# johnnyjana730/MVIN

Measured on AMD Instinct MI355X. Metric: (user,item) pairs scored/sec @ dim=64 hop=2 fan-out=32; % HBM roofline, higher is better.
Workload: dtype f32

## Files before the change

### mvin_amd/build.py

```python
import argparse
import hashlib
import os
import shutil
import subprocess
import sys

PKG_DIR = os.path.dirname(os.path.abspath(__file__))
CSRC = os.path.join(PKG_DIR, "csrc")
INCLUDE = os.path.join(os.path.dirname(PKG_DIR), "include")
LIB_PATH = os.path.join(PKG_DIR, "libmvin_hip.so")
STAMP_PATH = LIB_PATH + ".stamp"
OBJ_DIR = os.path.join(PKG_DIR, "_build")
SOURCES = ["mvin_kernels.hip", "mvin_fused.hip", "mvin_fused_split.hip", "mvin_fused_packed.hip", "mvin_fused_wpp.hip", "mvin_fused_agg.hip", "mvin_fused_agg32.hip", "mvin_fused_wpp_fold.hip", "mvin_fused_d16.hip", "mvin_fused_d32.hip", "mvin_tail.hip", "mvin_tail_flash.hip", "mvin_score_small.hip", "mvin_keyaddr.hip", "mvin_keyaddr_stream.hip", "mvin_keyaddr_grouped.hip", "mvin_keyaddr_dense.hip", "mvin_keyaddr_static.hip", "mvin_keyaddr_flash.hip", "mvin_keyaddr_wave.hip", "mvin_hoist.hip", "mvin_probe.hip", "mvin_group.hip", "mvin_order.hip", "mvin_topk.hip", "mvin_rank.hip", "mvin_segments.hip", "mvin_mmr.hip", "mvin_mips.hip", "mvin_resample.hip", "mvin_explore.hip", "mvin_ctr_metrics.hip", "mvin_ctr_delong.hip", "mvin_ctr_curve.hip", "mvin_ctr_rank_resample.hip","mvin_ctr_cluster.hip", "mvin_ctr_segments.hip", "mvin_ctr_calib.hip", "mvin_rank_head.hip", "mvin_mf.hip", "mvin_select_negatives.hip", "mvin_explain.hip", "mvin_explain_mem.hip", "mvin_prep.hip", "mvin_negatives.hip", "mvin_linear_mfma.hip", "mvin_entity_tables.hip", "mvin_bwd.hip", "mvin_grad_guard.hip",
           "mvin_abi_basic.hip", "mvin_abi_levels.hip", "mvin_abi_keyaddr.hip", "mvin_abi_score.hip", "mvin_abi_eval.hip", "mvin_abi_train.hip"]
HEADERS = ["mvin_common.h", "mvin_kernels.h", "mvin_launch.h", "mvin_fused_agg.h", "mvin_score_image.h", "mvin_ctr_bodies.h", "mvin_row_select.h", "mvin_rnd.h", "mvin_explain_mass.h", "mvin_rank_head_body.h",
           "mvin_workspaces.h", "mvin_score_plan.h", "mvin_abi_util.h", "mvin_entity_tables_plan.h", "mvin_l2_kernel_plan.h"]
VERSION_SCRIPT = os.path.join(CSRC, "libmvin_hip.map")
ARCH = "gfx950"
FLAGS = ["-O3", "-std=c++17", "-fPIC", "-fvisibility=hidden", "-shared", f"--offload-arch={ARCH}"]


def _hipcc():
    for cand in (os.environ.get("HIPCC"), shutil.which("hipcc"), "/opt/rocm/bin/hipcc"):
        if cand and os.path.exists(cand):
            return cand
    raise RuntimeError("hipcc not found (looked at $HIPCC, PATH, /opt/rocm/bin/hipcc)")


def _existing(names, base):
    return [os.path.join(base, n) for n in names if os.path.exists(os.path.join(base, n))]


def _digest():
    h = hashlib.sha256(" ".join(FLAGS).encode())
    for path in _existing(SOURCES + HEADERS, CSRC) + [os.path.join(INCLUDE, "mvin_hip.h"), VERSION_SCRIPT]:
        with open(path, "rb") as f:
            h.update(path.encode())
            h.update(f.read())
    return h.hexdigest()


def needs_build():
    if not os.path.exists(LIB_PATH) or not os.path.exists(STAMP_PATH):
        return True
    with open(STAMP_PATH) as f:
        return f.read().strip() != _digest()


def _obj_digest(src):
    h = hashlib.sha256(" ".join(FLAGS).encode())
    for path in [src] + _existing(HEADERS, CSRC) + [os.path.join(INCLUDE, "mvin_hip.h")]:
        with open(path, "rb") as f:
            h.update(f.read())
    return h.hexdigest()[:20]


def build(force=False, verbose=False, jobs=None):
    if not force and not needs_build():
        return LIB_PATH
    os.makedirs(OBJ_DIR, exist_ok=True)
    import fcntl
    with open(os.path.join(OBJ_DIR, ".lock"), "w") as lock:
        fcntl.flock(lock, fcntl.LOCK_EX)
        try:
            if not force and not needs_build():
                return LIB_PATH
            return _build_locked(force, verbose, jobs)
        finally:
            fcntl.flock(lock, fcntl.LOCK_UN)


def _build_locked(force, verbose, jobs):
    from concurrent.futures import ThreadPoolExecutor
    tmp_suffix = f".{os.getpid()}.tmp"
    hipcc = _hipcc()
    cflags = [f for f in FLAGS if f != "-shared"]
    todo, objs = [], []
    for src in _existing(SOURCES, CSRC):
        obj = os.path.join(OBJ_DIR, os.path.basename(src) + "." + _obj_digest(src) + ".o")
        objs.append(obj)
        if force or not os.path.exists(obj):
            todo.append((src, obj))

    def compile_one(job):
        src, obj = job
        cmd = [hipcc] + cflags + ["-c", f"-I{INCLUDE}", f"-I{CSRC}", src, "-o", obj + tmp_suffix]
        if verbose:
            print(" ".join(cmd), file=sys.stderr)
        res = subprocess.run(cmd, capture_output=True, text=True)
        if res.returncode != 0:
            raise RuntimeError(f"hipcc failed ({res.returncode}) on {src}:\n{res.stdout}\n{res.stderr}")
        if verbose and res.stderr:
            print(res.stderr, file=sys.stderr)
        os.replace(obj + tmp_suffix, obj)

    if todo:
        with ThreadPoolExecutor(max_workers=jobs or min(6, os.cpu_count() or 1)) as ex:
            list(ex.map(compile_one, todo))
    keep = set(objs)
    for f in os.listdir(OBJ_DIR):
        if os.path.join(OBJ_DIR, f) not in keep and not f.endswith(".tmp") and f != ".lock":
            os.remove(os.path.join(OBJ_DIR, f))
    cmd = [hipcc, "-shared", "-fPIC", f"--offload-arch={ARCH}", f"-Wl,--version-script={VERSION_SCRIPT}"] + objs + ["-o", LIB_PATH + tmp_suffix]
    res = subprocess.run(cmd, capture_output=True, text=True)
    if res.returncode != 0:
        raise RuntimeError(f"link failed ({res.returncode}):\n{res.stdout}\n{res.stderr}")
    os.replace(LIB_PATH + tmp_suffix, LIB_PATH)
    with open(STAMP_PATH, "w") as f:
        f.write(_digest())
    return LIB_PATH


if __name__ == "__main__":
    ap = argparse.ArgumentParser()
    ap.add_argument("--force", action="store_true")
    ap.add_argument("--verbose", action="store_true")
    a = ap.parse_args()
    print(build(force=a.force, verbose=a.verbose))
```

### mvin_amd/csrc/mvin_abi_keyaddr.hip

```cpp
#include "mvin_abi_util.h"

namespace mvin {
namespace abi {

int group_pairs_impl(const int64_t* users_i64, const int32_t* users_i32, int64_t B, int n_user, int32_t* workspace, int32_t* seg_user,
                     int32_t* seg_ptr, int32_t* nseg, int32_t* pair_index, void* stream, const int64_t* items64, unsigned max_id,
                     int32_t* item_rows) {
    const char* who = "mvin_group_pairs_by_user";
    if ((!users_i64 && !users_i32) || !workspace || !seg_user || !seg_ptr || !nseg || !pair_index)
        return fail(-1, "%s: null pointer", who);
    if (B <= 0 || B > 0x7fffffff || n_user <= 0) return fail(-2, "%s: bad sizes B=%lld n_user=%d", who, (long long)B, n_user);
    const GroupWs L(n_user, B);
    return hip_result(mvin::launch_group_pairs(users_i64, users_i32, B, n_user, workspace + L.counters(), workspace + L.offsets(),
                                               workspace + L.ranks(), seg_user, seg_ptr, nseg, pair_index, (hipStream_t)stream,
                                               reinterpret_cast<const int32_t*>(items64), 2, max_id, item_rows), who);
}

int flash_prepare_impl(const char* who, const float* entity_emb, const float* relation_kge, const float* w, const float* user_mlp_W, int n_entity,
                       int nR, int D, int P, float* ws, float* fold_ws, void* stream) {
    if (!entity_emb || !relation_kge || !user_mlp_W || !ws) return fail(-1, "%s: null pointer", who);
    if (n_entity <= 0 || nR <= 0 || D != 64 || P < 1 || P > 8) return fail(-2, "%s: n_entity=%d nR=%d D=%d P=%d", who, n_entity, nR, D, P);
    const RelWs L(n_entity, nR, D);
    if (int rc = build_entity_tables(who, entity_emb, n_entity, relation_kge, nR, ws + L.ER(), user_mlp_W, P + (w ? 1 : 0), ws + L.TW(),
                                     fold_ws ? fold_ws + FoldWs(n_entity, D).block() : nullptr, fold_ws, stream))
        return rc;
    if (w) return hip_result(mvin::launch_entity_dot(entity_emb, w, n_entity, D, ws + L.hs(), (hipStream_t)stream), who);
    return 0;
}

}
}

using namespace mvin::abi;

extern "C" {

int mvin_key_addressing_supported(int Nm, int D) {
    return (!bad_dim(D) && Nm > 0 && mvin::key_addr_nj(Nm, D) <= 16) ? 1 : 0;
}

static int key_addressing_impl(const char* who, const void* entity_emb, const float* V, const float* w,
                               const int32_t* const* mem_h, const int32_t* const* mem_r, const int32_t* const* mem_t,
                               const int32_t* uts, const int64_t* users64, const int32_t* users32, int P, int B, int Nm,
                               int D, int nR, int n_entity, int n_user, float* out, int64_t ldo, int table_bf16,
                               void* stream) {
    if (n_entity <= 0) return fail(-2, "%s: n_entity=%d", who, n_entity);
    if (uts && n_user <= 0) return fail(-2, "%s: n_user=%d", who, n_user);
    if (!entity_emb || !out || (!uts && !mem_h)) return fail(-1, "%s: null pointer", who);
    if (uts && !users64 && !users32) return fail(-1, "%s: user_triplet_set given without user ids", who);
    if (P < 0 || P > 8) return fail(-2, "%s: P=%d (0..8)", who, P);
    if (P == 0 && !w) return fail(-2, "%s: nothing to do (P == 0 and w == NULL)", who);
    if (P > 0 && (!V || nR <= 0 || (!uts && (!mem_r || !mem_t)))) return fail(-1, "%s: hops need V, mem_r, mem_t, nR", who);
    if (B <= 0 || Nm <= 0) return fail(-2, "%s: bad sizes B=%d Nm=%d", who, B, Nm);
    if (bad_dim(D)) return fail(-2, "%s: D=%d (need %%4==0, 4..%d)", who, D, MVIN_MAX_DIM);
    const int n_o = P + (w ? 1 : 0);
    if (ldo < (int64_t)n_o * D || (ldo & 3)) return fail(-2, "%s: ldo=%lld", who, (long long)ldo);
    mvin::KeyAddrArgs k{};
    k.E = entity_emb;
    k.V = V;
    k.w = w;
    k.uts = uts;
    k.users64 = users64;
    k.users32 = users32;
    k.n_user = n_user;
    k.n_entity = n_entity;
    const int nh = P > 0 ? P : 1;
    for (int i = 0; i < nh && !uts; ++i) {
        if (!mem_h[i]) return fail(-1, "%s: null mem_h[%d]", who, i);
        k.mem_h[i] = mem_h[i];
        if (i < P) {
            if (!mem_r[i] || !mem_t[i]) return fail(-1, "%s: null mem_r/mem_t[%d]", who, i);
            k.mem_r[i] = mem_r[i];
            k.mem_t[i] = mem_t[i];
        }
    }
    k.out = out;
    k.ldo = ldo;
    k.B = B;
    k.P = P;
    k.Nm = Nm;
    k.D = D;
    k.nR = nR;
    k.lpr_log2 = mvin::lpr_log2_for(D);
    k.table_bytes = (uint64_t)n_entity * D * (table_bf16 ? 2 : 4);
    if (!mvin::key_addr_stream_supported(k, table_bf16) && mvin::key_addr_nj(Nm, D) > 16)
        return fail(-3, "%s: unsupported shape Nm=%d D=%d (streaming kernel: Nm <= 64 and nR*D*4 <= 3072; "
                    "register-resident kernel: ceil(Nm / (64 / lanes per row)) <= 16)", who, Nm, D);
    return hip_result(mvin::launch_key_addr(k, table_bf16, (hipStream_t)stream), who);
}

int mvin_key_addressing_fwd(const void* entity_emb, const float* V, const float* w,
                            const int32_t* const* mem_h, const int32_t* const* mem_r,
                            const int32_t* const* mem_t, int P, int B, int Nm, int D, int nR, int n_entity,
                            float* out, int64_t ldo, int table_bf16, void* stream) {
    return key_addressing_impl("mvin_key_addressing_fwd", entity_emb, V, w, mem_h, mem_r, mem_t, nullptr, nullptr, nullptr, P,
                               B, Nm, D, nR, n_entity, 0, out, ldo, table_bf16, stream);
}

int mvin_key_addressing_users_fwd(const void* entity_emb, const float* V, const float* w, const int32_t* uts,
                                  const int64_t* users_i64, const int32_t* users_i32, int P, int B, int Nm, int D, int nR,
                                  int n_entity, int n_user, float* out, int64_t ldo, int table_bf16, void* stream) {
    return key_addressing_impl("mvin_key_addressing_users_fwd", entity_emb, V, w, nullptr, nullptr, nullptr, uts, users_i64,
                               users_i32, P, B, Nm, D, nR, n_entity, n_user, out, ldo, table_bf16, stream);
}

int mvin_group_pairs_by_user(const int64_t* users_i64, const int32_t* users_i32, int64_t B, int n_user, int32_t* workspace,
                             int32_t* seg_user, int32_t* seg_ptr, int32_t* nseg, int32_t* pair_index, void* stream) {
    return group_pairs_impl(users_i64, users_i32, B, n_user, workspace, seg_user, seg_ptr, nseg, pair_index, stream, nullptr, 0, nullptr);
}

int mvin_key_addressing_grouped_supported(int D, int P, int Nm, int nR) {
    return mvin::key_addr_grouped_supported(D, P, Nm, nR) ? 1 : 0;
}

int mvin_user_records_len(int P, int Nm, int nR) { return mvin::ka_rec_layout(P, Nm, nR).len; }

int mvin_user_records_supported(int D, int P, int Nm, int nR, int table_bf16) {
    return !table_bf16 && mvin::key_addr_static_supported(D, P, Nm, nR) ? 1 : 0;
}

int mvin_build_user_records(const int32_t* uts, int n_user, int P, int Nm, int nR, int n_entity, int32_t* records, void* stream) {
    const char* who = "mvin_build_user_records";
    if (!uts || !records) return fail(-1, "%s: null pointer", who);
    if (n_user <= 0 || n_entity <= 0) return fail(-2, "%s: bad sizes n_user=%d n_entity=%d", who, n_user, n_entity);
    if (mvin::ka_rec_layout(P, Nm, nR).len == 0) return fail(-3, "%s: no record form for P=%d Nm=%d nR=%d (P 1..8, Nm 1..256, nR 1..4096)", who, P, Nm, nR);
    return hip_result(mvin::launch_user_records(uts, n_user, P, Nm, nR, n_entity, records, (hipStream_t)stream), who);
}

int mvin_key_addressing_grouped_fwd(const void* entity_emb, const float* relation_kge, const float* w,
                                    const int32_t* uts, const int32_t* seg_user, const int32_t* seg_ptr,
                                    const int32_t* nseg_dev, const int32_t* pair_index, const int64_t* items_i64,
                                    const int32_t* items_i32, int nseg, int B, int P, int Nm, int D, int nR,
                                    int n_entity, int n_user, float* out, int64_t ldo, int table_bf16, void* stream) {
    return mvin_key_addressing_grouped_rec_fwd(entity_emb, relation_kge, w, uts, nullptr, seg_user, seg_ptr, nseg_dev, pair_index, items_i64,
                                               items_i32, nseg, B, P, Nm, D, nR, n_entity, n_user, out, ldo, table_bf16, stream);
}

size_t mvin_project_relations_elems(int n_entity, int nR, int D) {
    return n_entity > 0 && nR > 0 && D > 0 ? mvin::RelWs(n_entity, nR, D).elems() : 0;
}

int mvin_project_relations(const float* entity_emb, const float* relation_kge, const float* w, int n_entity, int nR, int D, float* ws,
                           void* stream) {
    const char* who = "mvin_project_relations";
    if (!entity_emb || !relation_kge || !ws) return fail(-1, "%s: null pointer", who);
    if (n_entity <= 0 || nR <= 0 || (D != 16 && D != 32 && D != 64 && D != 128)) return fail(-2, "%s: n_entity=%d nR=%d D=%d", who, n_entity, nR, D);
    const mvin::RelWs L(n_entity, nR, D);
    if (D == 64) {
        if (int rc = build_entity_tables(who, entity_emb, n_entity, relation_kge, nR, ws + L.ER(), nullptr, 0, nullptr, nullptr, nullptr, stream)) return rc;
    } else {
        float* RT = ws + L.RT();
        if (int rc = hip_result(mvin::launch_transpose_blocks(relation_kge, nR, D, RT, (hipStream_t)stream), who)) return rc;
        mvin_linear_args l{};
        l.src[0] = entity_emb;
        l.nsrc = 1;
        l.Dsrc = D;
        l.Dout = D;
        l.rows = n_entity;
        l.rows_per_group = 1;
        l.W = RT;
        l.w_zstride = (int64_t)L.DD;
        l.out = ws + L.ER();
        l.ldo = D;
        l.nz = nR;
        l.out_zstride = (int64_t)L.tab;
        if (int rc = mvin_linear_fwd(&l, stream)) return rc;
    }
    if (w) return hip_result(mvin::launch_entity_dot(entity_emb, w, n_entity, D, ws + L.hs(), (hipStream_t)stream), who);
    return 0;
}

int mvin_key_addressing_flash_supported(int D, int P, int Nm, int nR, int n_entity) {
    return mvin::key_addr_flash_supported(D, P, Nm, nR, n_entity) ? 1 : 0;
}

static int flash_nseg_bound(int64_t B, int n_user) { return (int)(B < (int64_t)n_user ? B : (int64_t)n_user); }

size_t mvin_key_addressing_flash_ws_elems(int64_t B, int n_user) {
    if (B <= 0 || n_user <= 0) return 0;
    return mvin::key_addr_flash_ws_elems(B, flash_nseg_bound(B, n_user));
}

size_t mvin_key_addressing_flash_tables_elems(int n_entity, int nR, int D, int P, int has_set) {
    if (n_entity <= 0 || nR <= 0 || D <= 0 || P < 0) return 0;
    return mvin::RelWs(n_entity, nR, D).flash_elems(P + (has_set ? 1 : 0));
}

int mvin_key_addressing_flash_prepare(const float* entity_emb, const float* relation_kge, const float* w, const float* user_mlp_W,
                                      int n_entity, int nR, int D, int P, float* ws, void* stream) {
    return flash_prepare_impl("mvin_key_addressing_flash_prepare", entity_emb, relation_kge, w, user_mlp_W, n_entity, nR, D, P, ws, nullptr,
                              stream);
}

int mvin_key_addressing_flash_fwd(const float* entity_emb, const float* ws, const int32_t* user_records, const int32_t* seg_user,
                                  const int32_t* seg_ptr, const int32_t* nseg_dev, const int32_t* pair_index, const int64_t* items_i64,
                                  const int32_t* items_i32, int64_t B, int P, int Nm, int D, int nR, int n_entity, int n_user, int has_set,
                                  const float* user_mlp_b, float* user_o, int32_t* sched_ws, void* stream) {
    const char* who = "mvin_key_addressing_flash_fwd";
    if (!entity_emb || !ws || !user_records || !seg_user || !seg_ptr || !pair_index || !user_o || !sched_ws)
        return fail(-1, "%s: null pointer", who);
    if ((items_i64 == nullptr) == (items_i32 == nullptr)) return fail(-1, "%s: exactly one of items_i64 / items_i32", who);
    if (B <= 0 || B >= (int64_t(1) << 31) || n_user <= 0 || n_entity <= 0 || nR <= 0)
        return fail(-2, "%s: bad sizes B=%lld n_user=%d n_entity=%d nR=%d", who, (long long)B, n_user, n_entity, nR);
    if (!mvin::key_addr_flash_supported(D, P, Nm, nR, n_entity))
        return fail(-3, "%s: unsupported shape D=%d P=%d Nm=%d nR=%d n_entity=%d (D = 64, 1 <= P <= 8, Nm <= 64, nR * n_entity < 2^31)", who,
                    D, P, Nm, nR, n_entity);
    mvin::KaFlashArgs k{};
    k.E = entity_emb;
    const mvin::RelWs L(n_entity, nR, D);
    k.ER = ws + L.ER();
    k.hs = has_set ? ws + L.hs() : nullptr;
    k.TW = ws + L.TW();
    k.records = user_records;
    k.seg_user = seg_user;
    k.seg_ptr = seg_ptr;
    k.nseg_dev = nseg_dev;
    k.pair_index = pair_index;
    k.items64 = items_i64;
    k.items32 = items_i32;
    k.bmlp = user_mlp_b;
    k.user_o = user_o;
    k.P = P;
    k.Nm = Nm;
    k.nR = nR;
    k.n_entity = n_entity;
    k.B = B;
    return hip_result(mvin::launch_key_addr_flash(k, flash_nseg_bound(B, n_user), has_set != 0, sched_ws, (hipStream_t)stream), who);
}

static int key_addressing_grouped_impl(const void* entity_emb, const float* relation_kge, const float* w,
                                        const int32_t* uts, const int32_t* user_records, const int32_t* seg_user,
                                        const int32_t* seg_ptr, const int32_t* nseg_dev, const int32_t* pair_index,
                                        const int64_t* items_i64, const int32_t* items_i32, int nseg, int B, int P, int Nm, int D,
                                        int nR, int n_entity, int n_user, float* out, int64_t ldo, int table_bf16, void* stream,
                                        const float* er_ws) {
    const char* who = "mvin_key_addressing_grouped_fwd";
    if (!entity_emb || !uts || !seg_user || !seg_ptr || !pair_index || !out) return fail(-1, "%s: null pointer", who);
    if ((items_i64 == nullptr) == (items_i32 == nullptr)) return fail(-1, "%s: exactly one of items_i64 / items_i32", who);
    if (P < 0 || P > 8) return fail(-2, "%s: P=%d (0..8)", who, P);
    if (P == 0 && !w) return fail(-2, "%s: nothing to do (P == 0 and w == NULL)", who);
    if (P > 0 && !relation_kge) return fail(-1, "%s: hops need relation_kge", who);
    if (nseg <= 0 || B <= 0 || Nm <= 0 || n_entity <= 0 || n_user <= 0 || nR <= 0)
        return fail(-2, "%s: bad sizes nseg=%d B=%d Nm=%d n_entity=%d n_user=%d nR=%d", who, nseg, B, Nm, n_entity, n_user, nR);
    const int n_o = P + (w ? 1 : 0);
    if (ldo < (int64_t)n_o * D || (ldo & 3)) return fail(-2, "%s: ldo=%lld", who, (long long)ldo);
    if (!mvin::key_addr_grouped_supported(D, P, Nm, nR))
        return fail(-3, "%s: unsupported shape D=%d P=%d Nm=%d nR=%d (D in {16,32,64,128}; rows + V tile must fit 160 KB "
                    "of LDS)", who, D, P, Nm, nR);
    mvin::KeyAddrGroupedArgs k{};
    k.E = entity_emb;
    k.R = relation_kge;
    k.w = w;
    k.uts = uts;
    k.seg_user = seg_user;
    k.seg_ptr = seg_ptr;
    k.nseg_dev = nseg_dev;
    k.pair_index = pair_index;
    k.items64 = items_i64;
    k.items32 = items_i32;
    k.out = out;
    k.ldo = ldo;
    k.nseg = nseg;
    k.P = P;
    k.Nm = Nm;
    k.D = D;
    k.nR = nR;
    k.n_entity = n_entity;
    k.records = user_records;
    if (er_ws) {
        const mvin::RelWs L(n_entity, nR, D);
        k.ER = er_ws + L.ER();
        k.hs = er_ws + L.hs();
    }
    return hip_result(mvin::launch_key_addr_grouped(k, table_bf16, (hipStream_t)stream), who);
}

int mvin_key_addressing_grouped_rec_fwd(const void* entity_emb, const float* relation_kge, const float* w,
                                        const int32_t* uts, const int32_t* user_records, const int32_t* seg_user,
                                        const int32_t* seg_ptr, const int32_t* nseg_dev, const int32_t* pair_index,
                                        const int64_t* items_i64, const int32_t* items_i32, int nseg, int B, int P, int Nm, int D,
                                        int nR, int n_entity, int n_user, float* out, int64_t ldo, int table_bf16, void* stream) {
    return key_addressing_grouped_impl(entity_emb, relation_kge, w, uts, user_records, seg_user, seg_ptr, nseg_dev, pair_index, items_i64,
                                       items_i32, nseg, B, P, Nm, D, nR, n_entity, n_user, out, ldo, table_bf16, stream, nullptr);
}

int mvin_key_addressing_grouped_er_supported(int D, int P, int Nm, int nR, int n_entity, int has_set) {
    return (D == 64 && mvin::key_addr_static_er_ok(P, Nm, nR, n_entity, has_set != 0)) ? 1 : 0;
}

int mvin_key_addressing_grouped_er_fwd(const void* entity_emb, const float* relation_kge, const float* w,
                                       const int32_t* uts, const int32_t* user_records, const float* er_ws, const int32_t* seg_user,
                                       const int32_t* seg_ptr, const int32_t* nseg_dev, const int32_t* pair_index,
                                       const int64_t* items_i64, const int32_t* items_i32, int nseg, int B, int P, int Nm, int D,
                                       int nR, int n_entity, int n_user, float* out, int64_t ldo, void* stream) {
    const char* who = "mvin_key_addressing_grouped_er_fwd";
    if (!user_records || !er_ws) return fail(-1, "%s: the gathered form needs the user records and the workspace of mvin_project_relations", who);
    if (!mvin_key_addressing_grouped_er_supported(D, P, Nm, nR, n_entity, w != nullptr))
        return fail(-3, "%s: unsupported shape D=%d P=%d Nm=%d nR=%d n_entity=%d", who, D, P, Nm, nR, n_entity);
    return key_addressing_grouped_impl(entity_emb, relation_kge, w, uts, user_records, seg_user, seg_ptr, nseg_dev, pair_index, items_i64,
                                       items_i32, nseg, B, P, Nm, D, nR, n_entity, n_user, out, ldo, 0, stream, er_ws);
}

}
```

### mvin_amd/csrc/mvin_abi_score.hip

```cpp
#include "mvin_abi_util.h"
#include "mvin_fused_agg.h"
#include "mvin_score_plan.h"

using namespace mvin::abi;
using mvin::DeepForm;
using mvin::ItemRowWord;
using mvin::KeyAddrForm;

namespace {

mvin::ScoreInputs score_inputs(const mvin_score_l2_args* a) {
    mvin::ScoreInputs in{};
    in.D = a->D, in.K = a->K, in.P = a->P, in.Nm = a->Nm, in.nR = a->n_relation, in.n_entity = a->n_entity, in.n_user = a->n_user, in.B = a->B;
    in.table_bf16 = a->table_bf16 != 0, in.fold_gather = a->fold_gather != 0, in.has_set = a->h_set_w != nullptr;
    in.uts = a->uts, in.group_ws = a->group_ws, in.user_records = a->user_records, in.ka_flash = a->ka_flash, in.ka_er = a->ka_er;
    in.fold_ws = a->fold_ws, in.enc_entity = a->enc_entity, in.enc_relation = a->enc_relation, in.W0 = a->W0, in.W1 = a->W1, in.W2 = a->W2;
    in.prj_tables = a->prj_tables, in.agg_tables = a->agg_tables, in.item_order_ws = a->item_order_ws;
    const int D = in.D, K = in.K, nR = in.nR, nE = in.n_entity;
    mvin::ScoreCaps& c = in.caps;
    c.flash = mvin::key_addr_flash_supported(D, in.P, in.Nm, nR, nE);
    c.er = mvin_key_addressing_grouped_er_supported(D, in.P, in.Nm, nR, nE, in.has_set) != 0;
    const mvin::L2Switches& sw = mvin::l2_switches();
    c.fold = mvin::fold_applies(D, K, nE, nR, in.B, sw);
    c.fold_gather = mvin::fold_gather_applies(D, K, nE, nR, in.B, sw);
    c.packed = mvin::fused_packed_supported(D, K);
    c.d32 = mvin::fused_d32_supported(D, K);
    c.prj = mvin::prj_applies(D, K, in.encoded(), nE, nR, in.B, sw);
    c.agg = mvin::agg_applies(D, K, nE, nR, in.B, sw);
    c.wpp = mvin::wpp_applies(D, K, nE, nR, in.B, a->enc_relation != nullptr, a->W1 != nullptr, a->W2 != nullptr, sw);
    static const bool item_rows_on = !(getenv("MVIN_ITEM_ROWS") && atoi(getenv("MVIN_ITEM_ROWS")) == 0);
    c.item_rows = item_rows_on;
    return in;
}

int project_v(const mvin_score_l2_args* a, void* stream) {
    const int D = a->D, nR = a->n_relation;
    mvin_linear_args l{};
    l.src[0] = reinterpret_cast<const float*>(a->entity_emb);
    l.ids[0] = reinterpret_cast<const int32_t*>(a->items);
    l.ids64 = 1;
    l.src_bf16 = a->table_bf16 ? 1 : 0;
    l.src_rows = a->n_entity;
    l.nsrc = 1;
    l.Dsrc = D;
    l.Dout = D;
    l.rows = a->B;
    l.W = a->relation_kge;
    l.rows_per_group = 1;
    l.out = a->V;
    l.ldo = (int64_t)nR * D;
    l.nz = nR;
    l.w_zstride = (int64_t)D * D;
    l.out_zstride = D;
    return mvin_linear_fwd(&l, stream);
}

int user_mlp(const mvin_score_l2_args* a, int n_o, void* stream) {
    mvin_linear_args u{};
    u.src[0] = a->o_cat;
    u.nsrc = 1;
    u.Dsrc = n_o * a->D;
    u.Dout = a->D;
    u.rows = a->B;
    u.W = a->user_mlp_W;
    u.bias = a->user_mlp_b;
    u.rows_per_group = 1;
    u.out = a->user_o;
    u.ldo = a->D;
    u.nz = 1;
    return mvin_linear_fwd(&u, stream);
}

int build_item_order(const mvin_score_l2_args* a, void* stream, const int32_t** order) {
    int32_t* ord = a->item_order_ws + mvin::order_ws_elems(a->B);
    if (int rc = mvin_order_by_key(a->items, nullptr, a->B, a->item_order_ws, ord, stream)) return rc;
    *order = ord;
    return 0;
}

}

extern "C" {

int mvin_score_l2_fwd(const mvin_score_l2_args* a, void* stream) {
    const char* who = "mvin_score_l2_fwd";
    if (!a) return fail(-1, "%s: null args", who);
    if (a->P < 1 || a->P > 8) return fail(-2, "%s: P=%d (1..8)", who, a->P);
    if ((!a->V && !(a->uts && a->group_ws)) || !a->o_cat || !a->parents || !a->nagg0 || !a->nagg1 || !a->user_o || !a->scores || !a->items)
        return fail(-1, "%s: null workspace / output / items", who);
    if (a->uts && !a->users) return fail(-1, "%s: user_triplet_set given without user ids", who);
    if (a->group_ws && !a->uts) return fail(-1, "%s: group_ws is for the users feed (uts + users)", who);
    const mvin::ScoreInputs in = score_inputs(a);
    const mvin::ScorePlan plan = mvin::plan_score(in);
    const int D = a->D, nR = a->n_relation, K = a->K, nE = a->n_entity, n_o = in.n_o();
    const float* E = reinterpret_cast<const float*>(a->entity_emb);
    const int64_t ldo = (int64_t)n_o * D;
    int rc = 0;

    int32_t* const item_rows = plan.item_row_word != ItemRowWord::None ? a->parents : nullptr;
    const unsigned item_max = (unsigned)(nE - 1);
    if (plan.item_row_word == ItemRowWord::OwnLaunch) {
        rc = hip_result(mvin::launch_item_rows(reinterpret_cast<const int32_t*>(a->items), 2, a->B, item_max, item_rows, (hipStream_t)stream), who);
        if (rc) return rc;
    }

    const mvin::GroupWs G(a->n_user, a->B);
    int32_t* const gws = a->group_ws;
    int32_t *seg_user = nullptr, *seg_ptr = nullptr, *nseg = nullptr, *pair_index = nullptr;
    if (plan.grouped()) {
        seg_user = gws + G.seg_user(), seg_ptr = gws + G.seg_ptr(), nseg = gws + G.nseg(), pair_index = gws + G.pair_index();
        rc = group_pairs_impl(a->users, nullptr, a->B, a->n_user, gws, seg_user, seg_ptr, nseg, pair_index, stream, a->items, item_max, item_rows);
        if (rc) return rc;
    }
    if (plan.project_v) {
        rc = project_v(a, stream);
        if (rc) return rc;
    }

    switch (plan.ka) {
        case KeyAddrForm::Flash:
            if (plan.fold_in_flash) {
                rc = fold_tables_check("mvin_fold_tables", E, a->enc_entity, a->enc_relation, a->W0, a->W1, a->W2, a->A0, a->Wmix, a->A1,
                                       plan.deep == DeepForm::Folded, K, D, nE, nR, a->fold_ws);
                if (rc) return rc;
                rc = fold_tables_block("mvin_fold_tables", a->t0, a->W0, a->b0, a->W1, a->b1, a->W2, a->b2, a->A0, a->a0, a->Wmix, a->bmix, a->A1,
                                       K, D, nE, a->fold_ws, stream);
                if (rc) return rc;
            }
            rc = flash_prepare_impl("mvin_key_addressing_flash_prepare", E, a->relation_kge, a->h_set_w, a->user_mlp_W, nE, nR, D, a->P,
                                    a->ka_flash, plan.fold_in_flash ? a->fold_ws : nullptr, stream);
            if (rc) return rc;
            if (!G.flash_sched_fits(mvin_key_addressing_flash_ws_elems(a->B, a->n_user)))
                return fail(-2, "%s: group_ws too small for the flash form's scheduling scratch", who);
            rc = mvin_key_addressing_flash_fwd(E, a->ka_flash, a->user_records, seg_user, seg_ptr, nseg, pair_index, a->items, nullptr, a->B,
                                               a->P, a->Nm, D, nR, nE, a->n_user, a->h_set_w != nullptr, a->user_mlp_b, a->user_o,
                                               gws + G.flash_sched(), stream);
            break;
        case KeyAddrForm::GatheredER:
            rc = mvin_project_relations(E, a->relation_kge, a->h_set_w, nE, nR, D, a->ka_er, stream);
            if (rc) return rc;
            rc = mvin_key_addressing_grouped_er_fwd(a->entity_emb, a->relation_kge, a->h_set_w, a->uts, a->user_records, a->ka_er, seg_user,
                                                    seg_ptr, nseg, pair_index, a->items, nullptr, (int)a->B, (int)a->B, a->P, a->Nm, D, nR, nE,
                                                    a->n_user, a->o_cat, ldo, stream);
            break;
        case KeyAddrForm::Records:
            rc = mvin_key_addressing_grouped_rec_fwd(a->entity_emb, a->relation_kge, a->h_set_w, a->uts, a->user_records, seg_user, seg_ptr, nseg,
                                                     pair_index, a->items, nullptr, (int)a->B, (int)a->B, a->P, a->Nm, D, nR, nE, a->n_user,
                                                     a->o_cat, ldo, a->table_bf16, stream);
            break;
        case KeyAddrForm::UsersFeed:
            rc = mvin_key_addressing_users_fwd(a->entity_emb, a->V, a->h_set_w, a->uts, a->users, nullptr, a->P, (int)a->B, a->Nm, D, nR, nE,
                                               a->n_user, a->o_cat, ldo, a->table_bf16, stream);
            break;
        case KeyAddrForm::PerPair:
            rc = mvin_key_addressing_fwd(a->entity_emb, a->V, a->h_set_w, a->mem_h, a->mem_r, a->mem_t, a->P, (int)a->B, a->Nm, D, nR, nE,
                                         a->o_cat, ldo, a->table_bf16, stream);
            break;
    }
    if (rc) return rc;
    if (plan.user_mlp) {
        rc = user_mlp(a, n_o, stream);
        if (rc) return rc;
    }

    const int32_t* const adj_e = plan.adj_encoded ? a->enc_entity : a->adj_entity;
    const int32_t* const adj_r = plan.adj_encoded ? a->enc_relation : a->adj_relation;
    const int32_t* order = nullptr;
    switch (plan.deep) {
        case DeepForm::FoldedGather:
            if (!plan.fold_in_flash)
                rc = mvin_fold_tables_ex(E, a->enc_entity, a->enc_relation, a->t0, a->W0, a->b0, a->W1, a->b1, a->W2, a->b2, a->A0, a->a0, a->Wmix,
                                         a->bmix, a->A1, 0, K, D, nE, nR, a->fold_ws, stream);
            if (rc) return rc;
            if (plan.build_order && (rc = build_item_order(a, stream, &order))) return rc;
            rc = mvin_score_l2_folded_gather_fwd(a->fold_ws, a->enc_entity, a->enc_relation, a->items, nullptr, order, a->t0, a->t1, a->user_o,
                                                 a->user_o, a->A1, a->a1, a->Wmix, a->B, K, D, nE, nR, a->item_emb, a->scores, a->sig, stream);
            break;
        case DeepForm::Folded:
            if (plan.fold_in_flash)
                rc = fold_tables_aggregates("mvin_fold_tables", a->enc_entity, a->enc_relation, a->t0, K, D, nE, nR, a->fold_ws, stream, item_rows);
            else
                rc = fold_tables_impl(E, a->enc_entity, a->enc_relation, a->t0, a->W0, a->b0, a->W1, a->b1, a->W2, a->b2, a->A0, a->a0, a->Wmix,
                                      a->bmix, a->A1, 1, K, D, nE, nR, a->fold_ws, stream, item_rows);
            if (rc) return rc;
            rc = mvin_score_l2_folded_fwd(a->fold_ws, a->enc_entity, a->enc_relation, a->items, nullptr, a->t0, a->t1, a->user_o, a->user_o, a->A1,
                                          a->a1, a->Wmix, a->B, K, D, nE, nR, a->nagg0, a->nagg1, a->item_emb, a->scores, a->sig, stream);
            break;
        case DeepForm::Aggregates:
        case DeepForm::Tables:
            rc = mvin_project_tables(E, a->W1, a->W2, a->b1, a->b2, a->A0, a->a0, a->t0 != nullptr, K, nE, D, a->prj_tables, stream);
            if (rc) return rc;
            if (plan.deep == DeepForm::Aggregates) {
                rc = mvin_entity_aggregates(a->prj_tables, a->enc_entity, a->enc_relation, a->t0, K, D, nE, nR, a->agg_tables, stream);
                if (rc) return rc;
                if (plan.build_order && (rc = build_item_order(a, stream, &order))) return rc;
                rc = mvin_gather_attn_l2_agg_fwd(a->prj_tables, a->agg_tables, a->enc_entity, a->enc_relation, a->items, 1, order, a->t0, a->t1,
                                                 a->user_o, (int)a->B, 1, K, D, nE, nR, a->nagg0, a->nagg1, stream);
            } else {
                if (plan.build_order && (rc = build_item_order(a, stream, &order))) return rc;
                rc = mvin_gather_attn_l2_prj_ordered_fwd(a->prj_tables, adj_e, adj_r, plan.adj_encoded ? 1 : 0, a->items, 1, order, a->t0, a->t1,
                                                         a->user_o, (int)a->B, 1, K, D, nE, nR, a->nagg0, a->nagg1, stream);
            }
            break;
        case DeepForm::Unprojected:
            rc = gather_attn_l2_impl(a->entity_emb, adj_e, adj_r, reinterpret_cast<const int32_t*>(a->items), 2, a->t0, a->t1, a->W1, a->W2, a->b1,
                                     a->b2, a->W1 ? a->user_o : nullptr, a->A0, a->a0, (int)a->B, 1, K, D, nE, nR, a->nagg0, a->nagg1, nullptr,
                                     nullptr, a->table_bf16, stream, plan.adj_encoded);
            break;
    }
    if (rc || !plan.tail) return rc;
    return mvin_l2_tail_fwd(a->entity_emb, a->items, nullptr, a->W0 ? a->user_o : nullptr, a->user_o, a->nagg0, a->nagg1, a->W0, a->b0, a->A0,
                            a->a0, a->A1, a->a1, a->Wmix, a->bmix, a->B, D, nE, a->item_emb, a->scores, a->sig, a->table_bf16, stream);
}

int mvin_score_small_supported(int D, int K, int P, int Nm, int nR) { return mvin::score_small_supported(D, K, P, Nm, nR) ? 1 : 0; }

int mvin_score_small_fwd(const mvin_score_l2_args* a, int group, void* stream) {
    const char* who = "mvin_score_small_fwd";
    if (!a) return fail(-1, "%s: null args", who);
    if (!mvin::score_small_supported(a->D, a->K, a->P, a->Nm, a->n_relation))
        return fail(-3, "%s: unsupported shape D=%d K=%d P=%d Nm=%d nR=%d (or V of nR relations beyond the workgroup's LDS)", who, a->D, a->K,
                    a->P, a->Nm, a->n_relation);
    if (a->depth < 0 || a->depth > 2) return fail(-2, "%s: depth=%d (1 or 2)", who, a->depth);
    const bool d1 = a->depth == 1;
    if (!a->entity_emb || !a->adj_entity || !a->relation_kge || !a->user_mlp_W || !a->A0 || (!d1 && !a->A1) || !a->Wmix || !a->items ||
        !a->user_o || !a->scores)
        return fail(-1, "%s: null table / weight / items / output", who);
    if ((a->W0 == nullptr) != (a->W1 == nullptr) || (!d1 && (a->W1 == nullptr) != (a->W2 == nullptr)))
        return fail(-1, "%s: W0 / W1 (/ W2) must be given together (User_orient) or not at all", who);
    if (a->uts ? !a->users : (!a->mem_h || !a->mem_r || !a->mem_t))
        return fail(-1, "%s: needs uts + users, or mem_h / mem_r / mem_t", who);
    if (a->B <= 0 || a->n_entity <= 0 || (a->uts && a->n_user <= 0)) return fail(-2, "%s: bad sizes B=%lld", who, (long long)a->B);
    const bool enc = a->enc_entity && a->enc_relation;
    if (enc && a->n_entity > (1 << 24)) return fail(-2, "%s: the encoded adjacency holds 24-bit ids", who);
    if (a->table_bf16) return fail(-3, "%s: fp32 entity table only", who);
    const uint64_t table_bytes = (uint64_t)a->n_entity * a->D * 4, adj_bytes = (uint64_t)a->n_entity * a->K * 4;
    if (table_bytes >= (1ull << 32) - 4096 || adj_bytes >= (1ull << 32) - 4096)
        return fail(-3, "%s: entity table / adjacency of 4 GiB or more (32-bit buffer offsets)", who);
    mvin::ScoreSmallArgs s{};
    s.E = a->entity_emb;
    s.adj_e = enc ? a->enc_entity : a->adj_entity;
    s.adj_r = enc ? a->enc_relation : a->adj_relation;
    s.R = a->relation_kge;
    s.w_h = a->h_set_w;
    s.Wu = a->user_mlp_W;
    s.bu = a->user_mlp_b;
    s.t0 = a->t0;
    s.t1 = a->t1;
    s.W0 = a->W0, s.b0 = a->b0, s.W1 = a->W1, s.b1 = a->b1, s.W2 = a->W2, s.b2 = a->b2;
    s.A0 = a->A0, s.a0 = a->a0, s.A1 = a->A1, s.a1 = a->a1, s.Wmix = a->Wmix, s.bmix = a->bmix;
    s.items = a->items;
    if (a->uts) {
        s.uts = a->uts;
        s.users = a->users;
    } else {
        for (int h = 0; h < a->P; ++h) {
            if (!a->mem_h[h] || !a->mem_r[h] || !a->mem_t[h]) return fail(-1, "%s: null ripple-set array of hop %d", who, h);
            s.mem_h[h] = a->mem_h[h], s.mem_r[h] = a->mem_r[h], s.mem_t[h] = a->mem_t[h];
        }
    }
    s.user_o = a->user_o, s.item_emb = a->item_emb, s.scores = a->scores, s.sig = a->sig;
    s.B = a->B;
    s.G = group;
    s.K = a->K, s.P = a->P, s.Nm = a->Nm, s.nR = a->n_relation, s.n_entity = a->n_entity, s.n_user = a->n_user > 0 ? a->n_user : 1;
    s.enc = enc ? 1 : 0;
    s.depth1 = d1 ? 1 : 0;
    s.table_bf16 = 0;
    s.table_bytes = table_bytes;
    s.adj_bytes = adj_bytes;
    return hip_result(mvin::launch_score_small(s, a->D, (hipStream_t)stream), who);
}

}
```

### mvin_amd/csrc/mvin_abi_util.h

```cpp
#pragma once
#include <cstdarg>
#include <cstdio>
#include <cstdlib>

#include "mvin_kernels.h"
#include "mvin_workspaces.h"

namespace mvin {
namespace abi {

int fail(int code, const char* fmt, ...);
int hip_result(hipError_t e, const char* what);
bool bad_dim(int D);
size_t geom_sum(int B, int K, int from, int to);

struct EntityTableList {
    const float* E;
    int n_entity;
    hipStream_t st;
    hipError_t err = hipSuccess;
    int n = 0;
    EntityTableJob jobs[kEtMaxJobs];
    void add(const float* W, int w_nk, float* out) {
        if (n == kEtMaxJobs) flush();
        jobs[n++] = EntityTableJob{W, out, w_nk};
    }
    void flush() {
        if (n > 0 && err == hipSuccess) err = launch_entity_tables(E, n_entity, jobs, n, st);
        n = 0;
    }
};

int build_entity_tables(const char* who, const float* E, int n_entity, const float* relation_kge, int nR, float* er, const float* user_mlp_W,
                        int n_o, float* tw, const float* fold_blk, float* fold_tabs, void* stream);

int gather_attn_l2_impl(const void* table, const int32_t* adj_entity, const int32_t* adj_relation, const int32_t* parent_ids, int pid_stride,
                        const float* t0, const float* t1, const float* W1, const float* W2, const float* b1, const float* b2, const float* q,
                        const float* A0, const float* a0, int B, int parents_per_pair, int K, int D, int n_entity, int nR, float* nagg0,
                        float* nagg1, float* probs_parent, float* probs_child, int table_bf16, void* stream, bool encoded = false,
                        bool prj = false, const int32_t* order = nullptr, const float* agg = nullptr);

int fold_tables_check(const char* who, const float* entity_emb, const int32_t* enc_entity, const int32_t* enc_relation, const float* W0,
                      const float* W1, const float* W2, const float* A0, const float* Wmix, const float* A1, int aggregates, int K, int D,
                      int n_entity, int nR, const float* ws);
int fold_tables_block(const char* who, const float* t0, const float* W0, const float* b0, const float* W1, const float* b1, const float* W2,
                      const float* b2, const float* A0, const float* a0, const float* Wmix, const float* bmix, const float* A1, int K, int D,
                      int n_entity, float* ws, void* stream);
int fold_tables_aggregates(const char* who, const int32_t* enc_entity, const int32_t* enc_relation, const float* t0, int K, int D, int n_entity,
                           int nR, float* ws, void* stream, const int32_t* rows_s = nullptr);
int fold_tables_impl(const float* entity_emb, const int32_t* enc_entity, const int32_t* enc_relation, const float* t0, const float* W0,
                     const float* b0, const float* W1, const float* b1, const float* W2, const float* b2, const float* A0, const float* a0,
                     const float* Wmix, const float* bmix, const float* A1, int aggregates, int K, int D, int n_entity, int nR, float* ws,
                     void* stream, const int32_t* rows_s);

int flash_prepare_impl(const char* who, const float* entity_emb, const float* relation_kge, const float* w, const float* user_mlp_W, int n_entity,
                       int nR, int D, int P, float* ws, float* fold_ws, void* stream);
int group_pairs_impl(const int64_t* users_i64, const int32_t* users_i32, int64_t B, int n_user, int32_t* workspace, int32_t* seg_user,
                     int32_t* seg_ptr, int32_t* nseg, int32_t* pair_index, void* stream, const int64_t* items64, unsigned max_id,
                     int32_t* item_rows);

}
}
```

### mvin_amd/csrc/mvin_fused_agg.hip

```cpp
#include "mvin_fused_agg.h"
#include "mvin_workspaces.h"

namespace mvin {

template <int K>
__global__ __launch_bounds__(kAggWaves * 64) void entity_aggregates_kernel(EntityAggArgs a) {
    constexpr int D = 64, SPL = K / 16;
    static_assert(K == 16 || K == 32 || K == 64, "K");
    extern __shared__ __attribute__((aligned(16))) float smem[];
    const int nRp = (a.nR + 3) & ~3;
    float* sT = smem;
    const int tid = threadIdx.x, lane = tid & 63, wave = tid >> 6;
    const int g = lane >> 4, c = lane & 15;
    unsigned* sLo = reinterpret_cast<unsigned*>(sT + nRp + wave * agg_list_words(K)) + g * (K + kAggPad);
    float* sLw = reinterpret_cast<float*>(reinterpret_cast<unsigned*>(sT + nRp + wave * agg_list_words(K)) + 4 * (K + kAggPad)) + g * (K + kAggPad);
    const bool att = a.t0 != nullptr;
    const float invK = 1.f / (float)K;
    const bool fast = agg_logit_table(a.t0, a.nR, sT, tid, lane);
    __syncthreads();

    const int tbytes = (int)a.table_bytes;
    const __amdgpu_buffer_rsrc_t tabS = __builtin_amdgcn_make_buffer_rsrc(const_cast<float*>(a.tabS), 0, tbytes, 0x00020000);
    const __amdgpu_buffer_rsrc_t tabG = __builtin_amdgcn_make_buffer_rsrc(const_cast<float*>(a.tabG), 0, tbytes, 0x00020000);
    const __amdgpu_buffer_rsrc_t selfS = __builtin_amdgcn_make_buffer_rsrc(const_cast<float*>(a.selfS), 0, a.selfS ? tbytes : 0, 0x00020000);
    const __amdgpu_buffer_rsrc_t selfG = __builtin_amdgcn_make_buffer_rsrc(const_cast<float*>(a.selfG), 0, tbytes, 0x00020000);
    const __amdgpu_buffer_rsrc_t adjE = __builtin_amdgcn_make_buffer_rsrc(const_cast<int32_t*>(a.adj_e), 0, (int)a.adj_bytes, 0x00020000);
    const __amdgpu_buffer_rsrc_t adjR = __builtin_amdgcn_make_buffer_rsrc(const_cast<int32_t*>(a.adj_r), 0, (int)a.adj_bytes, 0x00020000);
    const __amdgpu_buffer_rsrc_t outS = __builtin_amdgcn_make_buffer_rsrc(a.outS, 0, tbytes, 0x00020000);
    const __amdgpu_buffer_rsrc_t outG = __builtin_amdgcn_make_buffer_rsrc(a.outG, 0, tbytes, 0x00020000);
    const unsigned c16 = (unsigned)c * 16u;
    const unsigned n_entity = (unsigned)a.n_entity;
    const unsigned nquad = (n_entity + 3u) >> 2;

    const unsigned rows_s = a.rows_s ? (unsigned)*a.rows_s : n_entity;
    auto run = [&](auto fast_tag, auto bound_tag) {
        constexpr bool FAST = decltype(fast_tag)::value, BOUND = decltype(bound_tag)::value;
        for (unsigned quad = blockIdx.x * kAggWaves + wave; quad < nquad; quad += gridDim.x * kAggWaves) {
            const bool doS = !BOUND || __builtin_amdgcn_readfirstlane(quad * 4u < rows_s ? 1 : 0) != 0;
            const unsigned e = quad * 4u + (unsigned)g;
            const bool valid = e < n_entity;
            unsigned ce[SPL], cr[SPL];
            agg_load_slots<SPL>(adjE, adjR, valid ? (e * (unsigned)K + (unsigned)(SPL * c)) * 4u : kAggOob, ce, cr);
            const unsigned so = valid ? e * (unsigned)(D * 4) + c16 : kAggPadRow;
            const float4 sg = agg_row4(selfG, so);
            float4 ss = make_float4(0.f, 0.f, 0.f, 0.f);
            if (doS) ss = agg_row4(selfS, so);
            float wk[SPL];
            agg_row_weights<SPL, FAST>(cr, att, sT, (unsigned)(a.nR - 1), invK, wk);
            int cc = (int)(cr[0] >> 24);
            cc = valid ? (cc < 1 ? 1 : (cc > K ? K : cc)) : 0;
            __builtin_amdgcn_fence(__ATOMIC_RELEASE, "wavefront");
            __builtin_amdgcn_wave_barrier();
#pragma unroll
            for (int i = 0; i < SPL; ++i) {
                sLo[SPL * c + i] = ((cr[i] >> 16) & 0xFFu) ? (ce[i] & 0xFFFFFFu) * (unsigned)(D * 4) : kAggPadRow;
                sLw[SPL * c + i] = wk[i];
            }
            __builtin_amdgcn_fence(__ATOMIC_RELEASE, "wavefront");
            __builtin_amdgcn_wave_barrier();
            __builtin_amdgcn_fence(__ATOMIC_ACQUIRE, "wavefront");
            const int kmax = __builtin_amdgcn_readfirstlane(agg_xor32_imax(agg_xor16_imax(cc)));
            f32x2 s01 = {0.f, 0.f}, s23 = {0.f, 0.f}, g01 = {0.f, 0.f}, g23 = {0.f, 0.f};
            auto round4 = [&](int k0, auto s_tag) {
                constexpr bool S = decltype(s_tag)::value;
                const uint4 o4 = *reinterpret_cast<const uint4*>(sLo + k0);
                const float4 w4 = *reinterpret_cast<const float4*>(sLw + k0);
                const unsigned off[4] = {o4.x, o4.y, o4.z, o4.w};
                const float ws_[4] = {w4.x, w4.y, w4.z, w4.w};
                float4 r1[4], r2[4];
#pragma unroll
                for (int t = 0; t < 4; ++t) {
                    if constexpr (S) r1[t] = agg_row4(tabS, off[t] + c16);
                    r2[t] = agg_row4(tabG, off[t] + c16);
                }
#pragma unroll
                for (int t = 0; t < 4; ++t) {
                    const f32x2 w2 = {ws_[t], ws_[t]};
                    if constexpr (S) {
                        s01 = __builtin_elementwise_fma(w2, f32x2{r1[t].x, r1[t].y}, s01);
                        s23 = __builtin_elementwise_fma(w2, f32x2{r1[t].z, r1[t].w}, s23);
                    }
                    g01 = __builtin_elementwise_fma(w2, f32x2{r2[t].x, r2[t].y}, g01);
                    g23 = __builtin_elementwise_fma(w2, f32x2{r2[t].z, r2[t].w}, g23);
                }
            };
            if (doS)
                for (int k0 = 0; k0 < kmax; k0 += 4) round4(k0, std::true_type{});
            else
                for (int k0 = 0; k0 < kmax; k0 += 4) round4(k0, std::false_type{});
            const unsigned oo = valid ? e * (unsigned)(D * 4) + c16 : kAggOob;
            const u32x4 vs = {__float_as_uint(s01[0] + ss.x), __float_as_uint(s01[1] + ss.y), __float_as_uint(s23[0] + ss.z),
                              __float_as_uint(s23[1] + ss.w)};
            const u32x4 vg = {__float_as_uint(g01[0] + sg.x), __float_as_uint(g01[1] + sg.y), __float_as_uint(g23[0] + sg.z),
                              __float_as_uint(g23[1] + sg.w)};
            if (doS) __builtin_amdgcn_raw_buffer_store_b128(vs, outS, oo, 0, 0);
            __builtin_amdgcn_raw_buffer_store_b128(vg, outG, oo, 0, 0);
        }
    };
    if (a.rows_s) {
        if (fast) run(std::true_type{}, std::true_type{});
        else run(std::false_type{}, std::true_type{});
    } else {
        if (fast) run(std::true_type{}, std::false_type{});
        else run(std::false_type{}, std::false_type{});
    }
}

template <int K>
__global__ __launch_bounds__(kAggWaves * 64, K == 64 ? 3 : 4) void gather_attn_l2_agg_kernel(FusedL2Args a) {
    constexpr int D = 64, SPL = K / 16;
    static_assert(K == 16 || K == 32 || K == 64, "K");
    extern __shared__ __attribute__((aligned(16))) float smem[];
    const int nRp = (a.nR + 3) & ~3;
    float* sT = smem;
    const int tid = threadIdx.x, lane = tid & 63, wave = tid >> 6;
    const int g = lane >> 4, c = lane & 15;
    float* sUV = sT + nRp + wave * (16 * kAggUvLd + agg_list_words(K));
    unsigned* sLo = reinterpret_cast<unsigned*>(sUV + 16 * kAggUvLd) + g * (K + kAggPad);
    float* sLw = reinterpret_cast<float*>(reinterpret_cast<unsigned*>(sUV + 16 * kAggUvLd) + 4 * (K + kAggPad)) + g * (K + kAggPad);
    const bool att1 = a.t1 != nullptr;
    const float invK = 1.f / (float)K;
    const bool fold = a.fold != 0;
    const float c0 = fold ? 1.f : a.t0 != nullptr ? invK : 1.f;
    const bool fast = agg_logit_table(a.t1, a.nR, sT, tid, lane);
    __syncthreads();

    const unsigned tbytes = (unsigned)a.table_bytes;
    const __amdgpu_buffer_rsrc_t aggS = __builtin_amdgcn_make_buffer_rsrc(a.agg, 0, (int)tbytes, 0x00020000);
    const __amdgpu_buffer_rsrc_t aggG = __builtin_amdgcn_make_buffer_rsrc(reinterpret_cast<char*>(a.agg) + a.table_bytes, 0, (int)tbytes, 0x00020000);
    const __amdgpu_buffer_rsrc_t adjE = __builtin_amdgcn_make_buffer_rsrc(const_cast<int32_t*>(a.adj_e), 0, (int)a.adj_bytes, 0x00020000);
    const __amdgpu_buffer_rsrc_t adjR = __builtin_amdgcn_make_buffer_rsrc(const_cast<int32_t*>(a.adj_r), 0, (int)a.adj_bytes, 0x00020000);
    const __amdgpu_buffer_rsrc_t out0 = __builtin_amdgcn_make_buffer_rsrc(a.nagg0, 0, (int)(a.P * D * 4), 0x00020000);
    const __amdgpu_buffer_rsrc_t out1 = __builtin_amdgcn_make_buffer_rsrc(a.nagg1, 0, (int)(a.P * D * 4), 0x00020000);
    const unsigned c16 = (unsigned)c * 16u;
    if (c < kAggPad) {
        sLo[K + c] = kAggPadRow;
        sLw[K + c] = 0.f;
    }

    const int64_t nbatch = (a.P + 15) >> 4;
    const int64_t nwaves = (int64_t)gridDim.x * kAggWaves;
    auto run = [&](auto fast_tag) {
        constexpr bool FAST = decltype(fast_tag)::value;
        for (int64_t batch = (int64_t)blockIdx.x * kAggWaves + wave; batch < nbatch; batch += nwaves) {
            const int64_t p_base = batch << 4;
            int64_t pr = min(p_base + c, a.P - 1);
            if (a.order) pr = a.order[pr];
            const int x0c = fused_parent_id(a, pr);
            {
                const unsigned qoff = (unsigned)(pr / a.parents_per_pair) * (unsigned)(D * 4) + (unsigned)g * 16u;
                const char* qbase = reinterpret_cast<const char*>(a.q);
                float4 qb[4];
// ... 466 lines not shown
#pragma unroll
                    for (int nt = 0; nt < 4; ++nt) o2[nt] = f32x4{fmaxf(o2[nt][0], 0.f), fmaxf(o2[nt][1], 0.f), fmaxf(o2[nt][2], 0.f), fmaxf(o2[nt][3], 0.f)};
                };
                auto read_ob = [&]() {
#pragma unroll
                    for (int nt = 0; nt < 4; ++nt) ob[nt] = *reinterpret_cast<const f32x4*>(sUV + c * kAggUvLd + 16 * nt + 4 * g);
                };
                if (a.dbg & 2) late2(std::integral_constant<int, 0>{}), late2(std::integral_constant<int, 1>{}), late2(std::integral_constant<int, 2>{});
                else
                    chain(std::integral_constant<int, 3>{}, [&](auto j_) { constexpr int j = decltype(j_)::value; return j == 0 ? a.A1 : j == 1 ? a.Wm1 : a.Wm2; },
                          [&](auto j_) -> const f32x4 (&)[4] {
                              constexpr int j = decltype(j_)::value;
                              if constexpr (j == 0) return zb;
                              else if constexpr (j == 1) return ob;
                              else return o2;
                          },
                          [&](auto j_) -> f32x4 (&)[4] { if constexpr (decltype(j_)::value == 0) return o2; else return qm; },
                          [&](auto j_) {
                              if constexpr (decltype(j_)::value == 0) relu_o2(), read_ob();
                          }, late2);
                stamp(15, false);
                if constexpr (!PIPE) m0_load();
                stamp(16, true);
                if constexpr (!PIPE) {
                    if (a.user_o != a.q) uo_load();
                    else
#pragma unroll
                        for (int ntp = 0; ntp < 4; ++ntp) uor[ntp] = qb[ntp];
                }
                float part = 0.f;
#pragma unroll
                for (int ntp = 0; ntp < 4; ++ntp) {
                    const f32x4 uo = uor[ntp];
                    const f32x4 it4 = qm[ntp] + m0r[ntp];
                    if (a.item_emb && cvalid) *reinterpret_cast<f32x4*>(reinterpret_cast<char*>(a.item_emb) + 64 * ntp + (size_t)roff) = it4;
                    part += it4[0] * uo[0] + it4[1] * uo[1] + it4[2] * uo[2] + it4[3] * uo[3];
                }
                part = xor32_sum(xor16_sum(part));
                if (g == 0 && cvalid) {
                    a.scores[pr] = part;
                    if (a.sig) a.sig[pr] = 1.f / (1.f + expf(-part));
                }
                stamp(17, false);
            }
            __builtin_amdgcn_fence(__ATOMIC_RELEASE, "wavefront");
            __builtin_amdgcn_wave_barrier();
            __builtin_amdgcn_fence(__ATOMIC_ACQUIRE, "wavefront");
            if constexpr (TRACE) ++traced;
        }
    };
    if (fast) run(std::true_type{});
    else run(std::false_type{});
}

hipError_t fold_read_trace(long long* host_dst, size_t n) {
    const size_t have = sizeof(g_fold_trace) / sizeof(long long);
    return hipMemcpyFromSymbol(host_dst, HIP_SYMBOL(g_fold_trace), (n < have ? n : have) * sizeof(long long));
}

template <int K>
static hipError_t launch_fold_k(const FoldArgs& a, hipStream_t st) {
    static const bool pipe = !(getenv("MVIN_FOLD_PIPE") && atoi(getenv("MVIN_FOLD_PIPE")) == 0);
    static const bool trace = getenv("MVIN_FOLD_TRACE") != nullptr;
    static const int grid_cap = getenv("MVIN_FOLD_GRID") ? atoi(getenv("MVIN_FOLD_GRID")) : 0;
    static const int wgs = getenv("MVIN_FOLD_WGS") ? atoi(getenv("MVIN_FOLD_WGS")) : 0;
    using Kern = void (*)(FoldArgs);
    constexpr bool kTwoLists = fused_agg_lds_words(0, K) * sizeof(float) + (size_t)kAggWaves * agg_list_words(K) * sizeof(float) <= kLdsNoOptIn;
    auto kernel_of = [&](int mode) -> Kern {
        if (trace) {
            if constexpr (kTwoLists) {
                if (mode == 2) return score_l2_folded_kernel<K, 2, true>;
            }
            return mode ? (Kern)score_l2_folded_kernel<K, 1, true> : (Kern)score_l2_folded_kernel<K, 0, true>;
        }
        if constexpr (kTwoLists) {
            if (mode == 2) return score_l2_folded_kernel<K, 2, false>;
        }
        return mode ? (Kern)score_l2_folded_kernel<K, 1, false> : (Kern)score_l2_folded_kernel<K, 0, false>;
    };
    struct Plan {
        int dev, nR, per_cu;
        size_t lds;
        Kern kern;
    };
    static thread_local Plan plan{-1, -1, 0, 0, nullptr};
    int dev = 0;
    if (hipGetDevice(&dev) != hipSuccess) return hipGetLastError();
    if (plan.dev != dev || plan.nR != a.nR) {
        auto occupancy = [&](Kern k, size_t lds) {
            const int v = workgroups_per_cu(k, kAggWaves * 64, lds, 0);
            return v > 8 ? 8 : v;
        };
        const size_t lds1 = fused_agg_lds_bytes(a.nR, K), lds2 = lds1 + (size_t)kAggWaves * agg_list_words(K) * sizeof(float);
        const int mode1 = pipe ? 1 : 0;
        const int occ1 = occupancy(kernel_of(mode1), lds1);
        const int occ2 = pipe && kTwoLists && lds2 <= kLdsNoOptIn ? occupancy(kernel_of(2), lds2) : 0;
        const bool two = occ2 > 0 && occ2 >= occ1;
        plan.kern = kernel_of(two ? 2 : mode1);
        plan.lds = two ? lds2 : lds1;
        plan.per_cu = two ? occ2 : occ1 > 0 ? occ1 : 4;
        if (wgs > 0) plan.per_cu = wgs;
        plan.dev = dev, plan.nR = a.nR;
        if (getenv("MVIN_FOLD_REPORT"))
            fprintf(stderr, "score_l2_folded_kernel<%d>: mode %d, LDS %zu bytes per workgroup, %d workgroups per CU\n", K, two ? 2 : mode1, plan.lds, plan.per_cu);
    }
    const int64_t nbatch = (a.B + 15) >> 4;
    const int64_t want = (nbatch + kAggWaves - 1) / kAggWaves;
    int64_t grid = persistent_grid(want, plan.per_cu);
    if (grid_cap > 0 && grid_cap < grid) grid = grid_cap;
    plan.kern<<<(int)grid, kAggWaves * 64, plan.lds, st>>>(a);
    return hipGetLastError();
}

hipError_t launch_score_l2_folded(const float* agg, const float* M0, const int32_t* adj_e, const int32_t* adj_r, const int32_t* items, int pid_stride,
                                  const float* t1, const float* q, const float* user_o, const float* Wq, const float* bq, const float* Wv,
                                  const float* bv, const float* Wqm, const float* A1, const float* a1, const float* Wm1, const float* Wm2,
                                  const float* bm, float* item_emb, float* scores, float* sig, int64_t B, int K, int D, int nR, int n_entity,
                                  hipStream_t st) {
    FoldArgs f{};
    f.agg = agg, f.M0 = M0, f.adj_e = adj_e, f.adj_r = adj_r, f.items = items, f.pid_stride = pid_stride, f.t1 = t1, f.q = q, f.user_o = user_o;
    f.Wq = Wq, f.bq = bq, f.Wv = Wv, f.bv = bv, f.Wqm = Wqm, f.A1 = A1, f.a1 = a1, f.Wm1 = Wm1, f.Wm2 = Wm2, f.bm = bm;
    f.item_emb = item_emb, f.scores = scores, f.sig = sig, f.B = B, f.K = K, f.nR = nR, f.max_id = (unsigned)(n_entity - 1);
    f.table_bytes = (uint64_t)n_entity * (uint64_t)D * 4, f.adj_bytes = (uint64_t)n_entity * (uint64_t)K * 4;
    static const char* dbg = getenv("MVIN_FOLD_DBG");
    f.dbg = dbg ? atoi(dbg) : 0;
    if (D == 32) return launch_score_l2_folded_d32(f, st);
    switch (K) {
        case 16: return launch_fold_k<16>(f, st);
        case 32: return launch_fold_k<32>(f, st);
        case 64: return launch_fold_k<64>(f, st);
        default: return hipErrorInvalidValue;
    }
}

template <int K>
static hipError_t launch_entity_aggregates_k(const EntityAggArgs& a, hipStream_t st) {
    const size_t lds = ((size_t)((a.nR + 3) & ~3) + (size_t)kAggWaves * agg_list_words(K)) * sizeof(float);
    const int64_t nquad = ((int64_t)a.n_entity + 3) >> 2;
    const int64_t want = (nquad + kAggWaves - 1) / kAggWaves;
    entity_aggregates_kernel<K><<<(int)persistent_grid(want, 8), kAggWaves * 64, lds, st>>>(a);
    return hipGetLastError();
}

hipError_t launch_entity_aggregates(const EntityAggArgs& a, hipStream_t st) {
    if (a.D == 32) return launch_entity_aggregates_d32(a, st);
    switch (a.K) {
        case 16: return launch_entity_aggregates_k<16>(a, st);
        case 32: return launch_entity_aggregates_k<32>(a, st);
        case 64: return launch_entity_aggregates_k<64>(a, st);
        default: return hipErrorInvalidValue;
    }
}

__global__ void fold_prepare_kernel(const float* __restrict__ W0, const float* __restrict__ b0, const float* __restrict__ W1,
                                    const float* __restrict__ b1, const float* __restrict__ W2, const float* __restrict__ b2,
                                    const float* __restrict__ A0, const float* __restrict__ a0, const float* __restrict__ Wmix,
                                    const float* __restrict__ bmix, const float* __restrict__ A1, float c, int D, float* __restrict__ blk) {
    const int i = blockIdx.x, j = threadIdx.x;
    const FoldBlock L(D);
    if (j >= D) return;
    float s0 = 0.f, s1 = 0.f, s2 = 0.f, sm = 0.f;
    for (int k0 = 0; k0 < D; k0 += 8) {
        float av[8], mv[8], x0[8], x1[8], x2[8];
#pragma unroll
        for (int k = 0; k < 8; ++k) {
            av[k] = A0[(size_t)(k0 + k) * D + j];
            mv[k] = Wmix[(size_t)(k0 + k) * D + j];
            x0[k] = i < D ? W0[(size_t)i * D + k0 + k] : (b0 ? b0[k0 + k] : 0.f);
            x1[k] = i < D ? W1[(size_t)i * D + k0 + k] : (b1 ? b1[k0 + k] : 0.f);
            x2[k] = i < D ? W2[(size_t)i * D + k0 + k] : (b2 ? b2[k0 + k] : 0.f);
        }
#pragma unroll
        for (int k = 0; k < 8; ++k) {
            s0 = fmaf(x0[k], av[k], s0);
            s1 = fmaf(x1[k], av[k], s1);
            s2 = fmaf(x2[k], av[k], s2);
            sm = fmaf(x0[k], mv[k], sm);
        }
    }
    if (i < D) {
        const size_t ij = (size_t)i * D + j;
        blk[L.Wstack(0) + ij] = s1;
        blk[L.Wstack(1) + ij] = s2;
        blk[L.Wstack(2) + ij] = s0;
        blk[L.Wstack(3) + ij] = sm;
        blk[L.Wv() + ij] = fmaf(c, s2, s1);
        blk[L.Wq() + ij] = fmaf(c, s1, s0);
        if (D == 64 || D == 32) {
            const size_t o = (size_t)i * D + (size_t)(j & 15) * (D / 16) + (size_t)(j >> 4);
            blk[L.Wperm(0) + o] = fmaf(c, s1, s0);
            blk[L.Wperm(1) + o] = fmaf(c, s2, s1);
            blk[L.Wperm(2) + o] = sm;
            blk[L.Wperm(3) + o] = A1[ij];
            blk[L.Wperm(4) + o] = Wmix[L.DD + ij];
            blk[L.Wperm(5) + o] = Wmix[2 * L.DD + ij];
        }
    } else {
        const float av0 = a0 ? a0[j] : 0.f;
        blk[L.bv() + j] = fmaf(c, s2, s1) + av0;
        blk[L.bq() + j] = fmaf(c, s1, s0) + av0;
        blk[L.bm() + j] = (bmix ? bmix[j] : 0.f) + sm;
    }
}

hipError_t launch_fold_prepare(const float* W0, const float* b0, const float* W1, const float* b1, const float* W2, const float* b2, const float* A0,
                               const float* a0, const float* Wmix, const float* bmix, const float* A1, float c, int D, float* blk, hipStream_t st) {
    fold_prepare_kernel<<<D + 1, D < 64 ? 64 : D, 0, st>>>(W0, b0, W1, b1, W2, b2, A0, a0, Wmix, bmix, A1, c, D, blk);
    return hipGetLastError();
}

template <int K>
static hipError_t launch_agg_k(const FusedL2Args& a, hipStream_t st) {
    const size_t lds = fused_agg_lds_bytes(a.nR, K);
    const int v = workgroups_per_cu(gather_attn_l2_agg_kernel<K>, kAggWaves * 64, lds, 4);
    const int64_t nbatch = (a.P + 15) >> 4;
    const int64_t want = (nbatch + kAggWaves - 1) / kAggWaves;
    gather_attn_l2_agg_kernel<K><<<(int)persistent_grid(want, v > 8 ? 8 : v), kAggWaves * 64, lds, st>>>(a);
    return hipGetLastError();
}

hipError_t launch_gather_attn_l2_agg(const FusedL2Args& a, hipStream_t st) {
    switch (a.K) {
        case 16: return launch_agg_k<16>(a, st);
        case 32: return launch_agg_k<32>(a, st);
        case 64: return launch_agg_k<64>(a, st);
        default: return hipErrorInvalidValue;
    }
}

}
```

### mvin_amd/csrc/mvin_group.hip

```cpp
#include <cstdlib>

#include "mvin_kernels.h"

namespace mvin {

__device__ __forceinline__ int64_t clamp_user(int64_t u, int n_user) { return u < 0 ? 0 : (u >= n_user ? n_user - 1 : u); }

__device__ __forceinline__ int item_row_end(const int32_t* items, int64_t i, int stride, unsigned max_id) {
    const unsigned x = (unsigned)items[i * stride];
    return (int)(x < max_id ? x : max_id) + 1;
}
__device__ __forceinline__ int wave_imax(int v) {
#pragma unroll
    for (int o = 32; o > 0; o >>= 1) v = max(v, __shfl_xor(v, o, kWave));
    return v;
}
__device__ __forceinline__ int block_imax_256(int m) {
    __shared__ int sM[4];
    m = wave_imax(m);
    if ((threadIdx.x & 63) == 0) sM[threadIdx.x >> 6] = m;
    __syncthreads();
    return max(max(sM[0], sM[1]), max(sM[2], sM[3]));
}

constexpr int kItemRowsBlocks = 64;
__global__ __launch_bounds__(256) void item_rows_kernel(const int32_t* __restrict__ items, int stride, int64_t B, unsigned max_id,
                                                        int32_t* __restrict__ item_rows) {
    int m = 0;
    for (int64_t i = (int64_t)blockIdx.x * blockDim.x + threadIdx.x; i < B; i += (int64_t)gridDim.x * blockDim.x)
        m = max(m, item_row_end(items, i, stride, max_id));
    m = block_imax_256(m);
    if (threadIdx.x == 0) atomicMax(item_rows, m);
}

hipError_t launch_item_rows(const int32_t* items, int item_stride, int64_t B, unsigned max_id, int32_t* item_rows, hipStream_t st) {
    if (hipError_t e = hipMemsetAsync(item_rows, 0, sizeof(int32_t), st); e != hipSuccess) return e;
    const int blocks = (int)((B + 255) / 256 < kItemRowsBlocks ? (B + 255) / 256 : kItemRowsBlocks);
    item_rows_kernel<<<blocks, 256, 0, st>>>(items, item_stride, B, max_id, item_rows);
    return hipGetLastError();
}

__global__ __launch_bounds__(256) void group_count_kernel(const int64_t* __restrict__ u64, const int32_t* __restrict__ u32, int64_t B,
                                                          int n_user, int32_t* __restrict__ count, int32_t* __restrict__ rank,
                                                          const int32_t* __restrict__ items, int item_stride, unsigned max_id,
                                                          int32_t* __restrict__ block_rows) {
    int m = 0;
    for (int64_t i = (int64_t)blockIdx.x * blockDim.x + threadIdx.x; i < B; i += (int64_t)gridDim.x * blockDim.x) {
        rank[i] = atomicAdd(count + clamp_user(u64 ? u64[i] : (int64_t)u32[i], n_user), 1);
        if (block_rows) m = max(m, item_row_end(items, i, item_stride, max_id));
    }
    if (block_rows) {
        m = block_imax_256(m);
        if (threadIdx.x == 0) block_rows[blockIdx.x] = m;
    }
}

__device__ __forceinline__ void block_scan2(int c, int s, int* sC, int* sS, int& ec, int& es, int& totC, int& totS) {
    const int lane = threadIdx.x & 63, wave = threadIdx.x >> 6;
    int ic = c, is = s;
#pragma unroll
    for (int o = 1; o < 64; o <<= 1) {
        const int tc = __shfl_up(ic, o, kWave), ts = __shfl_up(is, o, kWave);
        if (lane >= o) {
            ic += tc;
            is += ts;
        }
    }
    if (lane == 63) {
        sC[wave] = ic;
        sS[wave] = is;
    }
    __syncthreads();
    int wc = 0, ws = 0;
    totC = 0;
    totS = 0;
#pragma unroll
    for (int w = 0; w < 16; ++w) {
        const int a = sC[w], b = sS[w];
        if (w < wave) {
            wc += a;
            ws += b;
        }
        totC += a;
        totS += b;
    }
    ec = wc + ic - c;
    es = ws + is - s;
}

constexpr int kScanTile = 16384;
__global__ __launch_bounds__(1024) void group_scan_kernel(const int32_t* __restrict__ count, int n_user, int64_t B,
                                                          int32_t* __restrict__ offs, int32_t* __restrict__ seg_user,
                                                          int32_t* __restrict__ seg_ptr, int32_t* __restrict__ nseg,
                                                          const int32_t* __restrict__ block_rows, int nblocks,
                                                          int32_t* __restrict__ item_rows) {
    extern __shared__ int sCnt[];
    int* sSeg = sCnt + min(n_user, kScanTile);
    __shared__ int sC[16], sS[16], sRows[16];
    const int tid = threadIdx.x;
    if (item_rows) {
        int m = 0;
        for (int b = tid; b < nblocks; b += 1024) m = max(m, block_rows[b]);
        m = wave_imax(m);
        if ((tid & 63) == 0) sRows[tid >> 6] = m;
    }
    int carryC = 0, carryS = 0;
    for (int t0 = 0; t0 < n_user; t0 += kScanTile) {
        const int n = min(kScanTile, n_user - t0);
        __syncthreads();
        for (int u0 = tid; u0 < n; u0 += 8 * 1024) {
            int v[8];
#pragma unroll
            for (int j = 0; j < 8; ++j) v[j] = u0 + j * 1024 < n ? count[t0 + u0 + j * 1024] : 0;
#pragma unroll
            for (int j = 0; j < 8; ++j)
                if (u0 + j * 1024 < n) sCnt[u0 + j * 1024] = v[j];
        }
        __syncthreads();
        const int per = ((n + 1023) / 1024) | 1;
        const int u0 = min(tid * per, n), u1 = min(u0 + per, n);
        int c = 0, s = 0;
        for (int u = u0; u < u1; ++u) {
            const int v = sCnt[u];
            c += v;
            s += v > 0 ? 1 : 0;
        }
        int ec, es, totC, totS;
        block_scan2(c, s, sC, sS, ec, es, totC, totS);
        ec += carryC;
        es += carryS;
        for (int u = u0; u < u1; ++u) {
            const int v = sCnt[u];
            sCnt[u] = ec;
            sSeg[u] = v > 0 ? es : -1;
            es += v > 0 ? 1 : 0;
            ec += v;
        }
        carryC += totC;
        carryS += totS;
        __syncthreads();
        for (int u = tid; u < n; u += 1024) {
            const int o = sCnt[u], sg = sSeg[u];
            offs[t0 + u] = o;
            if (sg >= 0) {
                seg_user[sg] = t0 + u;
                seg_ptr[sg] = o;
            }
        }
    }
    if (tid == 0) {
        nseg[0] = carryS;
        seg_ptr[carryS] = carryC;
        if (item_rows) {
            int m = 0;
            for (int w = 0; w < 16; ++w) m = max(m, sRows[w]);
            item_rows[0] = m;
        }
    }
}

__global__ __launch_bounds__(1024) void group_small_kernel(const int64_t* __restrict__ u64, const int32_t* __restrict__ u32, int64_t B,
                                                           int n_user, int32_t* __restrict__ seg_user, int32_t* __restrict__ seg_ptr,
                                                           int32_t* __restrict__ nseg, int32_t* __restrict__ pair_index,
                                                           const int32_t* __restrict__ items, int item_stride, unsigned max_id,
                                                           int32_t* __restrict__ item_rows) {
    extern __shared__ int sCount[];
    __shared__ int sC[16], sS[16], sRows[16];
    const int tid = threadIdx.x;
    for (int u = tid; u < n_user; u += 1024) sCount[u] = 0;
    __syncthreads();
    constexpr int UN = 16;
    for (int64_t base = 0; base < B; base += 1024 * UN) {
        int u[UN];
#pragma unroll
        for (int j = 0; j < UN; ++j) {
            const int64_t i = base + j * 1024 + tid;
            u[j] = i < B ? (int)clamp_user(u64 ? u64[i] : (int64_t)u32[i], n_user) : -1;
        }
#pragma unroll
        for (int j = 0; j < UN; ++j)
            if (u[j] >= 0) atomicAdd(&sCount[u[j]], 1);
    }
    if (item_rows) {
        int m = 0;
        for (int64_t i = tid; i < B; i += 1024) m = max(m, item_row_end(items, i, item_stride, max_id));
        m = wave_imax(m);
        if ((tid & 63) == 0) sRows[tid >> 6] = m;
    }
    __syncthreads();
    const int per = ((n_user + 1023) / 1024) | 1;
    const int u0 = min(tid * per, n_user), u1 = min(u0 + per, n_user);
    int c = 0, s = 0;
    for (int u = u0; u < u1; ++u) {
        const int v = sCount[u];
        c += v;
        s += v > 0 ? 1 : 0;
    }
    int ec, es, totC, totS;
    block_scan2(c, s, sC, sS, ec, es, totC, totS);
    for (int u = u0; u < u1; ++u) {
        const int v = sCount[u];
        sCount[u] = ec;
        if (v > 0) {
            seg_user[es] = u;
            seg_ptr[es] = ec;
            ++es;
        }
        ec += v;
    }
    if (tid == 0) {
        nseg[0] = totS;
        seg_ptr[totS] = totC;
        if (item_rows) {
            int m = 0;
            for (int w = 0; w < 16; ++w) m = max(m, sRows[w]);
            item_rows[0] = m;
        }
    }
    __syncthreads();
    for (int64_t base = 0; base < B; base += 1024 * UN) {
        int u[UN], pos[UN];
#pragma unroll
        for (int j = 0; j < UN; ++j) {
            const int64_t i = base + j * 1024 + tid;
            u[j] = i < B ? (int)clamp_user(u64 ? u64[i] : (int64_t)u32[i], n_user) : -1;
        }
#pragma unroll
        for (int j = 0; j < UN; ++j) pos[j] = u[j] >= 0 ? atomicAdd(&sCount[u[j]], 1) : 0;
#pragma unroll
        for (int j = 0; j < UN; ++j)
            if (u[j] >= 0) pair_index[pos[j]] = (int32_t)(base + j * 1024 + tid);
    }
}

__global__ void group_scatter_kernel(const int64_t* __restrict__ u64, const int32_t* __restrict__ u32, int64_t B, int n_user,
                                     const int32_t* __restrict__ offs, const int32_t* __restrict__ rank,
                                     int32_t* __restrict__ pair_index) {
    for (int64_t i = (int64_t)blockIdx.x * blockDim.x + threadIdx.x; i < B; i += (int64_t)gridDim.x * blockDim.x) {
        pair_index[offs[clamp_user(u64 ? u64[i] : (int64_t)u32[i], n_user)] + rank[i]] = (int32_t)i;
    }
}

constexpr int64_t kGroupSmallMaxB = 32768;
constexpr size_t kGroupSmallMaxLds = 150 * 1024;

hipError_t launch_group_pairs(const int64_t* u64, const int32_t* u32, int64_t B, int n_user, int32_t* count, int32_t* offs,
                              int32_t* rank, int32_t* seg_user, int32_t* seg_ptr, int32_t* nseg, int32_t* pair_index, hipStream_t st,
                              const int32_t* items, int item_stride, unsigned max_id, int32_t* item_rows) {
    if (!items) item_rows = nullptr;
    static const int force = getenv("MVIN_GROUP_SMALL") ? atoi(getenv("MVIN_GROUP_SMALL")) : -1;
    const size_t lds = (size_t)n_user * sizeof(int32_t);
    const bool small = lds <= kGroupSmallMaxLds && (force < 0 ? B <= kGroupSmallMaxB : force == 1);
    if (small) {
        if (hipError_t e = grant_lds(group_small_kernel, lds, 48 * 1024); e != hipSuccess) return e;
        group_small_kernel<<<1, 1024, lds, st>>>(u64, u32, B, n_user, seg_user, seg_ptr, nseg, pair_index, items, item_stride, max_id, item_rows);
        return hipGetLastError();
    }
    hipError_t e = hipMemsetAsync(count, 0, (size_t)n_user * sizeof(int32_t), st);
    if (e != hipSuccess) return e;
    const int blocks = (int)((B + 255) / 256 < 2048 ? (B + 255) / 256 : 2048);
    group_count_kernel<<<blocks, 256, 0, st>>>(u64, u32, B, n_user, count, rank, items, item_stride, max_id, item_rows ? pair_index : nullptr);
    {
        const size_t scan_lds = (size_t)2 * (n_user < kScanTile ? n_user : kScanTile) * sizeof(int32_t);
        e = grant_lds(group_scan_kernel, scan_lds, 48 * 1024);
        if (e != hipSuccess) return e;
        group_scan_kernel<<<1, 1024, scan_lds, st>>>(count, n_user, B, offs, seg_user, seg_ptr, nseg, pair_index, blocks, item_rows);
    }
    group_scatter_kernel<<<blocks, 256, 0, st>>>(u64, u32, B, n_user, offs, rank, pair_index);
    return hipGetLastError();
}

}
```

### mvin_amd/csrc/mvin_kernels.h

```cpp
#pragma once
#include <hip/hip_runtime.h>
#include <stdint.h>

#include "../../include/mvin_hip.h"
#include "mvin_common.h"
#include "mvin_launch.h"
#include "mvin_l2_kernel_plan.h"

namespace mvin {

struct GatherAttnArgs {
    int gather;
    int table_bf16;
    const void* table;
    const int32_t* adj_e;
    const int32_t* adj_r;
    const int32_t* node_ids;
    const float* neigh;
    const int32_t* rel_ids;
    const float* rel_score;
    const float* self_vec;
    const float* Wc;
    const float* c_child;
    const float* Wagg;
// ... 191 lines not shown
    const int32_t* adj_r;
    const int32_t* parent_ids;
    const float* t0;
    const float* t1;
    const float* W1;
    const float* W2;
    const float* q;
    const float* b1;
    const float* b2;
    const float* A0;
    const float* a0;
    float* nagg0;
    float* nagg1;
    float* probs_parent;
    float* probs_child;
    int64_t P;
    uint64_t table_bytes;
    uint64_t adj_bytes;
    int parents_per_pair, K, nR, lpn_log2;
    int pid_stride;
    unsigned max_id;
    int dbg;
    const int32_t* order;
    float* agg;
    int fold;
    int prj;
};

__device__ __forceinline__ int fused_parent_id(const FusedL2Args& a, int64_t i) {
    const unsigned v = (unsigned)a.parent_ids[i * a.pid_stride];
    return (int)(v < a.max_id ? v : a.max_id);
}

struct EltArgs {
    int mode;
    int64_t n;
    float* x;
    float* y;
    float* z;
    float* w;
    float* accum;
    float alpha, beta, beta1, beta2, eps;
    int D, N;
};

struct WgradArgs {
    mvin_linear_args lin;
    const float* dY;
    int64_t ldy, dy_zstride;
    const float* mask;
    int64_t ldm, mask_zstride;
    float* dW;
    int64_t dw_zstride;
    float* db;
    int64_t db_zstride;
    int IB;
};

struct AggBwdArgs {
    int gather;
    const float* table;
    const int32_t* adj_e;
    const int32_t* adj_r;
    const int32_t* node_ids;
    const float* child;
    const int32_t* rel_ids;
    const float* probs;
    const float* rel_score;
    int skip_zero;
    const float* dvec;
    float* dtable;
    float* dchild;
    float* dT;
    int64_t T;
    int K, D, nR, lpr_log2;
};

struct KeyAddrBwdArgs {
    KeyAddrArgs f;
    const float* dout;
    float* dE;
    float* dV;
    float* dw;
    float l2;
    const float* Rk;
    const void* items;
    int items64;
    int dw_rep;
    int dv_lds;
    float* reg_accum;
};

hipError_t launch_eltwise(const EltArgs& a, hipStream_t st);
hipError_t launch_l2_adam_multi(const mvin_param_seg* segs, int nseg, int64_t total, float* g, float* mo, float* vo,
                                float* accum, int apply_adam, float lr_t, const float* lr_dev, float b1, float b2,
                                float eps, hipStream_t st);
hipError_t launch_l2_adam_multi_guarded(const mvin_param_seg* segs, int nseg, int64_t total, float* g, float* mo, float* vo,
                                        float* accum, int apply_adam, const mvin_guard_state* guard, float b1, float b2,
                                        float eps, hipStream_t st);
hipError_t launch_grad_guard(const mvin_param_seg* segs, int nseg, int64_t total, const float* g,
                             const mvin_guard_item* items, int nitems, mvin_guard_partial* partials,
                             const float* lr_table, int lr_table_len, mvin_guard_state* state, int grid_cap,
                             hipStream_t st);
hipError_t launch_scatter_add_rows(float* dtable, const int32_t* ids, int ids64, const float* x, int64_t rows, int D,
                                   float alpha, hipStream_t st);
hipError_t launch_linear_wgrad(WgradArgs a, hipStream_t st);
hipError_t launch_linear_wgrad_multi(const WgradArgs* probs, int n, hipStream_t st);
hipError_t launch_agg_bwd(const AggBwdArgs& a, hipStream_t st);
hipError_t launch_rel_score_bwd(const float* rel, const float* urh_w, const float* dT, int nR, int D, float* drel,
                                float* durh, hipStream_t st);
hipError_t launch_key_addr_bwd(const KeyAddrBwdArgs& a, hipStream_t st);

inline int lpr_log2_for(int D) {
    int l = 0;
    while ((4 << l) < D) ++l;
    return l;
}

hipError_t launch_expand(const int32_t* adj_e, const int32_t* adj_r, const int64_t* items64,
                         const int32_t* items32, int B, int K, int levels, int n_entity,
                         int32_t* ent_out, int32_t* rel_out, hipStream_t st);
hipError_t launch_rel_score(const float* rel, const float* urh_w, int nR, int D, float* t,
                            hipStream_t st);
hipError_t launch_linear(const mvin_linear_args& a, hipStream_t st);
constexpr size_t kLdsLimit = 160 * 1024;
inline size_t linear_valu_lds_bytes(const mvin_linear_args& a) {
    return (size_t)kTM * ((a.sum_sources ? 1 : a.nsrc) * a.Dsrc + 4) * sizeof(float);
}
inline size_t gather_attn_lds_bytes(int D, int K) {
    return (size_t)2 * kTM * (D + 4) * sizeof(float) + (size_t)4 * K * sizeof(int2);
}
bool linear_takes_valu(const mvin_linear_args& a);
bool linear_mfma_supported(const mvin_linear_args& a);
hipError_t launch_linear_mfma(const mvin_linear_args& a, hipStream_t st);
hipError_t launch_gather_attn(const GatherAttnArgs& a, hipStream_t st);
hipError_t launch_ripple(const RippleArgs& a, hipStream_t st);
hipError_t launch_sample_adjacency(const int64_t* indptr, const int32_t* dst, const int32_t* rel, int n_entity,
                                   int K, uint64_t seed, int32_t* adj_e, int32_t* adj_r, hipStream_t st);
hipError_t launch_ripple_build(const RippleBuildArgs& a, hipStream_t st);
int key_addr_nj(int Nm, int D);
bool key_addr_grouped_supported(int D, int P, int Nm, int nR);
hipError_t launch_key_addr_grouped(const KeyAddrGroupedArgs& a, int table_bf16, hipStream_t st);
bool key_addr_wave16_supported(int D, int P, int Nm, int nR);
bool key_addr_wave16_applies(const KeyAddrGroupedArgs& a);
hipError_t launch_key_addr_wave16(const KeyAddrGroupedArgs& a, int table_bf16, hipStream_t st);
bool key_addr_dense_supported(int D, int P, int Nm, int nR);
hipError_t launch_key_addr_dense(const KeyAddrGroupedArgs& a, int table_bf16, hipStream_t st);
KaRecLayout ka_rec_layout(int P, int Nm, int nR);
hipError_t launch_user_records(const int32_t* uts, int n_user, int P, int Nm, int nR, int n_entity, int32_t* out, hipStream_t st);
bool key_addr_static_supported(int D, int P, int Nm, int nR);
bool key_addr_static_applies(const KeyAddrGroupedArgs& a, int table_bf16);
hipError_t launch_key_addr_static(const KeyAddrGroupedArgs& a, hipStream_t st);
bool key_addr_flash_supported(int D, int P, int Nm, int nR, int n_entity);
size_t key_addr_flash_ws_elems(int64_t B, int nseg_bound);
hipError_t launch_key_addr_flash(const KaFlashArgs& a, int nseg_bound, bool has_set, int32_t* sched_ws, hipStream_t st);
hipError_t kas_read_trace(long long* host_dst, size_t n);
hipError_t kaf_read_trace(long long* host_dst, size_t n);
hipError_t fold_read_trace(long long* host_dst, size_t n);
hipError_t launch_key_addr(const KeyAddrArgs& a, int table_bf16, hipStream_t st);
bool key_addr_stream_supported(const KeyAddrArgs& a, int table_bf16);
hipError_t launch_key_addr_stream(const KeyAddrArgs& a, int table_bf16, hipStream_t st);
hipError_t launch_move_rows(void* table, const int32_t* ids, int64_t n, int row_bytes, void* rows, bool scatter,
                            hipStream_t st);
hipError_t launch_shard_space_ids(const void* ids, bool is64, int64_t n, int world, int n_local, void* out, hipStream_t st);
hipError_t launch_row_softmax(const float* x, int64_t rows, int n, float* out, hipStream_t st);
hipError_t launch_mix_urv(const float* neigh, const float* rel, const float* user, const float* logits, int64_t nodes, int N, int K,
                          int D, float* out, float* probs, hipStream_t st);
hipError_t launch_gather_mix(const GatherMixArgs& a, hipStream_t st);
struct ScoreSmallArgs {
    const void* E;
    const int32_t* adj_e;
    const int32_t* adj_r;
    const float* R;
    const float* w_h;
    const float* Wu;
    const float* bu;
    const float* t0;
    const float* t1;
    const float *W0, *b0, *W1, *b1, *W2, *b2;
    const float *A0, *a0, *A1, *a1, *Wmix, *bmix;
    const int64_t* items;
    const int32_t* mem_h[4];
    const int32_t* mem_r[4];
    const int32_t* mem_t[4];
    const int32_t* uts;
    const int64_t* users;
    float* user_o;
    float* item_emb;
    float* scores;
    float* sig;
    int64_t B;
    int G;
    int K, P, Nm, nR, n_entity, n_user, enc, table_bf16;
    int depth1;
    int dbg;
    uint64_t table_bytes;
    uint64_t adj_bytes;
};
bool score_small_supported(int D, int K, int P, int Nm, int nR);
int score_small_group(int D, int K, int P, int Nm, int nR, int has_hset, int64_t B);
hipError_t launch_score_small(ScoreSmallArgs a, int D, hipStream_t st);
hipError_t small_read_trace(long long* host_dst, size_t n);

bool l2_tail_supported(int D);
hipError_t launch_l2_tail(const TailArgs& a, int D, hipStream_t st);
bool l2_tail_flash_applies(const TailArgs& a, int D);
hipError_t launch_l2_tail_flash(const TailArgs& a, hipStream_t st);
hipError_t launch_gather_attn_l2(const FusedL2Args& a, int D, int table_bf16, hipStream_t st);
hipError_t launch_gather_probe_l2(const void* table, const int32_t* ids1, const int32_t* ids2, int64_t n_parents, int K,
                                  int D, int table_bf16, float* sums, hipStream_t st);
hipError_t launch_group_pairs(const int64_t* u64, const int32_t* u32, int64_t B, int n_user, int32_t* count, int32_t* offs,
                              int32_t* rank, int32_t* seg_user, int32_t* seg_ptr, int32_t* nseg, int32_t* pair_index, hipStream_t st,
                              const int32_t* items = nullptr, int item_stride = 1, unsigned max_id = 0, int32_t* item_rows = nullptr);
hipError_t launch_item_rows(const int32_t* items, int item_stride, int64_t B, unsigned max_id, int32_t* item_rows, hipStream_t st);
hipError_t launch_count_ids(const int32_t* ids, int64_t n, int nbins, float* out, hipStream_t st);
bool topk_rows_supported(int k);
hipError_t launch_topk_rows(const float* scores, int64_t rows, int64_t n, int64_t ld, const int32_t* cand_ids, int64_t col_offset,
                            const int64_t* excl_ptr, const int32_t* excl_ids, const int32_t* carry_ids, const float* carry_vals, int k,
                            int32_t* out_ids, float* out_vals, hipStream_t st);
hipError_t launch_rank_positives(const float* scores, int64_t rows, int64_t n, int64_t ld, const int32_t* cand_ids, int64_t col_offset,
                                 const int64_t* excl_ptr, const int32_t* excl_ids, const int64_t* pos_ptr, const int32_t* pos_ids,
                                 int32_t* out_counts, float* out_vals, int32_t* out_eligible, hipStream_t st);
int segments_wave_cap();
hipError_t launch_topk_segments(const float* scores, int64_t total, const int64_t* seg_ptr, int64_t n_seg, const int32_t* ids,
                                const int64_t* excl_ptr, const int32_t* excl_ids, int k, int64_t max_len, int form, int32_t* out_pos,
                                float* out_vals, int32_t* out_ids, int64_t* status, hipStream_t st);
hipError_t launch_rank_segments(const float* scores, int64_t total, const int64_t* seg_ptr, int64_t n_seg, const int32_t* ids,
                                const int64_t* excl_ptr, const int32_t* excl_ids, const int64_t* q_ptr, const int32_t* q_pos,
                                int64_t n_q, int64_t max_len, int form, int32_t* out_counts, float* out_vals, int32_t* out_eligible,
                                int64_t* status, hipStream_t st);
int mmr_max_len();
hipError_t launch_row_inv_norms(const float* feat, int64_t n_rows, int D, int64_t ld, float eps, float* out, hipStream_t st);
hipError_t launch_mmr_segments(const float* scores, int64_t total, const int64_t* seg_ptr, int64_t n_seg, const int32_t* ids,
                               const int64_t* excl_ptr, const int32_t* excl_ids, const float* feat, int64_t n_rows, int D, int64_t ld,
                               const float* row_scale, float lam, int k, int64_t max_len, int form, int32_t* out_pos, float* out_vals,
                               int32_t* out_ids, float* out_mmr, float* out_pen, float* out_simsum, int64_t* status, hipStream_t st);
int mips_topk_max_k();
int mips_max_splits();
bool mips_dim_ok(int D);
bool mips_topk_supported(int k, int D);
int mips_resolve_splits(int64_t nq, int64_t n, int splits);
int64_t mips_topk_ws_bytes(int64_t nq, int64_t n, int k, int splits);
hipError_t launch_mips_scores(const float* q, int64_t nq, const float* feat, int64_t n_rows, int D, int64_t ld, const float* q_scale,
                              const float* row_scale, const int32_t* cand_ids, int64_t col_offset, int64_t n, float* out, int64_t ldo,
                              hipStream_t st);
hipError_t launch_mips_topk(const float* q, int64_t nq, const float* feat, int64_t n_rows, int D, int64_t ld, const float* q_scale,
                            const float* row_scale, const int32_t* cand_ids, int64_t col_offset, int64_t n, const int64_t* excl_ptr,
                            const int32_t* excl_ids, int k, int splits, void* ws, int32_t* out_ids, float* out_vals, hipStream_t st);
hipError_t launch_mean_rows_segments(const float* feat, int64_t n_rows, int D, int64_t ld, const int64_t* seg_ptr, int64_t n_seg,
                                     const int32_t* ids, int64_t total, int group, float* out, hipStream_t st);
int resample_max_cols();
hipError_t launch_resample_sums(const double* vals, int64_t n_rows, int n_cols, int64_t ld, int mode, uint64_t seed, int64_t first,
                                int64_t n_rep, int max_groups, double* sums, int32_t* counts, hipStream_t st);
int64_t ctr_counts_ws_bytes(int64_t n_seg, int64_t seg_len);
hipError_t launch_ctr_counts(const float* scores, const int32_t* labels, int64_t n_seg, int64_t seg_len, int64_t ld, void* ws,
                             int64_t* out, hipStream_t st);
hipError_t launch_ctr_counts_segments(const float* scores, const int32_t* labels, int64_t total, const int64_t* seg_ptr, int64_t n_seg,
                                      float threshold, int64_t max_len, int form, int64_t* out, int64_t* status, hipStream_t st);
int64_t ctr_placements_ws_bytes(int64_t n);
hipError_t launch_ctr_placements(const float* scores, const int32_t* labels, int64_t n, void* ws, int64_t* place, int64_t* counts,
                                 hipStream_t st);
hipError_t ctr_sort_classes(const float* scores, const int32_t* labels, int64_t n, void* ws, int64_t* counts, int bad_slot, int* cur,
                            hipStream_t st);
int placement_moments_max_models();
hipError_t launch_placement_moments(const int64_t* place, int64_t ld, int K, const int32_t* labels, int64_t n, int max_groups,
                                    uint64_t* cross, int64_t* sums, int64_t* counts, hipStream_t st);
int placement_cluster_gram_words(int K);
hipError_t launch_placement_cluster_moments(const int64_t* place, int64_t ld, int K, const int32_t* labels, int64_t n,
                                            const int32_t* order, const int64_t* seg_ptr, int64_t n_clusters, int max_groups,
                                            int64_t* csum, uint64_t* gram, int64_t* totals, hipStream_t st);
int segment_sums_max_cols();
hipError_t launch_segment_sums_f64(const double* vals, int64_t n, int M, int64_t ld, const int32_t* order, const int64_t* seg_ptr,
                                   int64_t n_clusters, double* out, hipStream_t st);
int64_t ctr_tails_ws_bytes(int64_t n);
hipError_t launch_ctr_tails(const float* scores, const int32_t* labels, int64_t n, void* ws, int32_t* tails, int64_t* counts,
                            hipStream_t st);
int64_t ctr_operating_points_ws_bytes(int64_t n);
hipError_t launch_ctr_operating_points(const int32_t* tails, const float* scores, const int32_t* labels, int64_t n, void* ws,
                                       int max_groups, float* thr, int64_t* cells, double* ap_sum, hipStream_t st);
int ctr_threshold_counts_max();
hipError_t launch_ctr_threshold_counts(const float* scores, const int32_t* labels, int64_t n, const float* thresholds, int T,
                                       int max_groups, int64_t* out, int64_t* counts, hipStream_t st);
hipError_t launch_resample_multiplicities(int64_t n_units, uint64_t seed, int64_t first, int64_t n_rep, int32_t* mult, int64_t ld,
                                          hipStream_t st);
int64_t ctr_rank_image_ws_bytes(int64_t n);
hipError_t launch_ctr_rank_image(const int32_t* tails, const int32_t* labels, const int32_t* units, int64_t n, void* ws,
                                 int32_t* pos_row, int32_t* image, hipStream_t st);
int ctr_rank_resample_max_cuts();
int64_t ctr_rank_resample_ws_bytes(int64_t n, int64_t n_rep);
hipError_t launch_ctr_rank_resample(const int32_t* image, int64_t n, const int32_t* mult, int64_t ld, int64_t n_units, int64_t n_rep,
                                    const int64_t* cut_pos, int n_cuts, int max_groups, void* ws, int64_t* out, double* ap_sum,
                                    hipStream_t st);
int64_t ctr_calib_ws_bytes(int64_t n_seg, int64_t seg_len);
hipError_t launch_ctr_calib(const float* logits, const int32_t* labels, int64_t n_seg, int64_t seg_len, int64_t ld, double a, double b,
                            double y0, double y1, const float* edges, int n_bins, int max_groups, void* ws, double* out_sums,
                            int64_t* out_counts, int64_t* out_bins, hipStream_t st);
bool sample_negatives_supported(int n_item);
hipError_t launch_sample_negatives(const int64_t* excl_ptr, const int32_t* excl_ids, const int32_t* counts, const int64_t* out_ptr,
                                   int n_user, int n_item, const uint32_t* alias_tab, const uint32_t* mask_bits, uint64_t seed,
                                   uint64_t round, int32_t* out, int64_t* status,
                                   hipStream_t st);
hipError_t launch_rank_head(const float* user_o, const float* item_emb, const float* valid, const float* offset, int64_t n_groups,
                            int G, int D, int mode, float scale, float* scores, float* dscore, float* du, float* di,
                            float* loss_accum, int64_t* counts,
                            hipStream_t st);
hipError_t launch_mf_head(const float* U, const float* V, int64_t n_user, int64_t n_item, const int64_t* users, const int64_t* items,
                          const float* valid, const float* labels, int64_t n_groups, int G, int D, int mode, float scale, float reg,
                          float* scores, float* dscore, float* du, float* di, float* loss_accum, int64_t* counts, int grid_cap,
                          hipStream_t st);
hipError_t launch_mf_scores(const float* U, const float* V, int64_t n_user, int64_t n_item, const int64_t* users, const int64_t* items,
                            int64_t B, int D, float* logits, float* probs, hipStream_t st);
hipError_t launch_sparse_adam_rows(float* x, float* m, float* v, int64_t n_rows, int D, const int64_t* keys, const int32_t* order,
                                   const float* grads, const float* valid, int64_t n, float lr_t, float b1, float b2, float eps,
                                   int64_t* status, int grid_cap, hipStream_t st);
int explain_paths_max_k();
hipError_t launch_explain_paths(const float* imp0, const float* imp1, const int32_t* rel0, const int32_t* ent1, const int32_t* rel1,
                                const int32_t* ent2, int64_t B, int K, int top, int n_relation, int32_t* out_paths,
                                int64_t* out_mass, int32_t* out_slot, int32_t* out_distinct, int64_t* out_total, int64_t* rel_mass,
                                hipStream_t st);
struct ExplainMemArgs {
    const float* entity_emb;
    const float* V;
    const float* w_h;
    const int32_t* uts;
    const long long* users;
    const float* G;
    const float* mlp_bias;
    const float* item_final;
    int64_t B;
    int P, Nm, D, nR, n_entity, n_user, top;
    int32_t* out_mem;
    long long* out_mass;
    float* out_contrib;
    int32_t* out_slot;
    int32_t* out_distinct;
    long long* out_total;
    float* out_block;
    float* out_bias;
    float* out_probs;
    float* out_slot_contrib;
    unsigned long long* rel_mass;
};
int explain_memories_max_nm();
hipError_t launch_explain_memories(const ExplainMemArgs& a, hipStream_t st);
hipError_t launch_select_negatives(const float* scores, const int64_t* items, const float* valid, const int64_t* group_key,
                                   int64_t n_groups, int Gp, int n_neg, int shortlist, uint64_t seed, uint64_t round,
                                   int64_t* out_items, float* out_valid, float* out_scores, int64_t* counts,
                                   hipStream_t st);
int64_t kg_explore_ws_bytes(int n_entity, int64_t M);
hipError_t launch_kg_field(const int64_t* eptr, const int32_t* edst, const int32_t* erel, int n_entity, int64_t M,
                           const int32_t* seeds, int64_t n_seed, int hops, void* ws, uint32_t* field_bits, int64_t* out_counts,
                           hipStream_t st);
hipError_t launch_kg_explore(const int64_t* eptr, const int32_t* edst, const int32_t* erel, int n_entity, int64_t M,
                             const int32_t* adj_entity, const int32_t* adj_relation, int K, const int32_t* seeds, int64_t n_seed,
                             int hops, void* ws, uint32_t* explored_bits, int64_t* out_counts, hipStream_t st);
size_t order_ws_elems(int64_t B);
hipError_t launch_order_by_key(const int64_t* k64, const int32_t* k32, int64_t B, int32_t* ws, int32_t* order, hipStream_t st);
hipError_t launch_gather_attn_l2_wpp(const FusedL2Args& a, hipStream_t st);
hipError_t launch_entity_aggregates(const EntityAggArgs& a, hipStream_t st);
hipError_t launch_fold_prepare(const float* W0, const float* b0, const float* W1, const float* b1, const float* W2, const float* b2, const float* A0,
                               const float* a0, const float* Wmix, const float* bmix, const float* A1, float c, int D, float* blk, hipStream_t st);
hipError_t launch_l2_tail_fold(const TailFoldArgs& a, hipStream_t st);
hipError_t launch_score_l2_folded(const float* agg, const float* M0, const int32_t* adj_e, const int32_t* adj_r, const int32_t* items, int pid_stride,
                                  const float* t1, const float* q, const float* user_o, const float* Wq, const float* bq, const float* Wv,
                                  const float* bv, const float* Wqm, const float* A1, const float* a1, const float* Wm1, const float* Wm2,
                                  const float* bm, float* item_emb, float* scores, float* sig, int64_t B, int K, int D, int nR, int n_entity,
                                  hipStream_t st);
hipError_t launch_gather_attn_l2_agg(const FusedL2Args& a, hipStream_t st);
hipError_t launch_gather_attn_l2_d32(const FusedL2Args& a, int table_bf16, hipStream_t st, bool encoded = false);
hipError_t launch_gather_attn_l2_d16(const FusedL2Args& a, int table_bf16, hipStream_t st);
hipError_t launch_gather_attn_l2_split(const FusedL2Args& a, int D, int table_bf16, hipStream_t st);
hipError_t split_read_trace(long long* host_dst, size_t n);
bool key_addr_static_er_ok(int P, int Nm, int nR, int n_entity, bool has_set);
hipError_t launch_transpose_blocks(const float* R, int nR, int D, float* RT, hipStream_t st);
constexpr int kEtMaxJobs = 24;
struct EntityTableJob {
    const float* W;
    float* out;
    int w_nk;
};
hipError_t launch_entity_tables(const float* E, int n_entity, const EntityTableJob* jobs, int njobs, hipStream_t st);
hipError_t launch_entity_dot(const float* E, const float* w, int n, int D, float* out, hipStream_t st);
hipError_t launch_prj_prepare(const float* W1, const float* W2, const float* b1, const float* b2, const float* A0, const float* a0,
                              float c, int D, float* blk, hipStream_t st);
hipError_t pack_read_prof(long long* host_dst, size_t n);
hipError_t launch_gather_attn_l2_packed(const FusedL2Args& a, int D, int table_bf16, hipStream_t st);
hipError_t launch_encode_adjacency(const int32_t* adj_e, const int32_t* adj_r, int n_entity, int K, int32_t* cnt,
                                   int32_t* enc_e, int32_t* enc_r, hipStream_t st);
hipError_t ka_read_trace(long long* host_dst, size_t n);

}
```

### mvin_amd/csrc/mvin_keyaddr_flash.hip

```cpp
#include <cstdlib>
#include <type_traits>

#include "mvin_kernels.h"

namespace mvin {

typedef float f32x4 __attribute__((ext_vector_type(4)));

constexpr int kFlashChunk = 64;
constexpr int kFlashWaves = 4;

__global__ void ka_flash_slots_kernel(const int32_t* __restrict__ seg_ptr, const int32_t* __restrict__ nseg_dev, int nseg_bound,
                                      int32_t* __restrict__ slot_seg) {
    const int nseg = nseg_dev ? min(*nseg_dev, nseg_bound) : nseg_bound;
    for (int s = blockIdx.x * blockDim.x + threadIdx.x; s < nseg; s += gridDim.x * blockDim.x) {
        const int p0 = seg_ptr[s], p1 = seg_ptr[s + 1];
        const int first = p0 / kFlashChunk + s;
        const int nch = (p1 - p0 + kFlashChunk - 1) / kFlashChunk;
        for (int c = 0; c < nch; ++c) slot_seg[first + c] = s;
    }
}

#define KAF_FENCE() __builtin_amdgcn_sched_barrier(0)

__device__ float g_kaf_no_bias[64];
__device__ long long g_kaf_trace[64 * 16];

extern __shared__ __attribute__((aligned(16))) int32_t sKafRec[];

template <int NMT, bool HAS_SET, bool PF, bool TRACE = false>
__global__ __launch_bounds__(kFlashWaves * 64, 2) void key_addr_flash_kernel(KaFlashArgs a, KaRecLayout RL) {
    constexpr int D = 64;
    __shared__ f32x4 sUo0[kFlashWaves][4][64];
    const int lane = threadIdx.x & 63, l16 = lane & 15, q16 = lane >> 4;
    f32x4 (*myUo0)[64] = sUo0[threadIdx.x >> 6];
    const int P = a.P, NmP = RL.NmP;
    const unsigned emax = (unsigned)(a.n_entity - 1);
    const float* __restrict__ E = a.E;
    const float* __restrict__ bias = a.bmlp;
    const size_t tw_stride = (size_t)a.n_entity * D;

    struct Rows {
        float4 v[NMT][4];
    };
    auto issue_u = [&](int mt, const int (&hr)[NMT], Rows& R) {
        const f32x4* src = reinterpret_cast<const f32x4*>(a.ER + (size_t)(unsigned)max(hr[mt], 0) * D) + q16;
#pragma unroll
        for (int nt = 0; nt < 4; ++nt) {
            const f32x4 v = src[4 * nt];
            R.v[mt][nt] = make_float4(v[0], v[1], v[2], v[3]);
        }
    };
    auto issue_t = [&](int mt, const float* __restrict__ tab, const int4 (&ids)[NMT], Rows& R) {
        const int id[4] = {ids[mt].x, ids[mt].y, ids[mt].z, ids[mt].w};
#pragma unroll
        for (int i = 0; i < 4; ++i)
            R.v[mt][i] = reinterpret_cast<const float4*>(tab + (size_t)(unsigned)max(id[i], 0) * D)[l16];
    };
    auto reads_tile = [&](bool two, int mt, const Rows& R, const f32x4 (&p0)[NMT], const f32x4 (&p1)[NMT], f32x4 (&u0)[4], f32x4 (&u1)[4]) {
        if (two) {
#pragma unroll
            for (int i = 0; i < 4; ++i) {
                const float t[4] = {R.v[mt][i].x, R.v[mt][i].y, R.v[mt][i].z, R.v[mt][i].w};
#pragma unroll
                for (int nt = 0; nt < 4; ++nt) u0[nt] = __builtin_amdgcn_mfma_f32_16x16x4f32(t[nt], p0[mt][i], u0[nt], 0, 0, 0);
#pragma unroll
                for (int nt = 0; nt < 4; ++nt) u1[nt] = __builtin_amdgcn_mfma_f32_16x16x4f32(t[nt], p1[mt][i], u1[nt], 0, 0, 0);
            }
        } else {
#pragma unroll
            for (int i = 0; i < 4; ++i) {
                const float t[4] = {R.v[mt][i].x, R.v[mt][i].y, R.v[mt][i].z, R.v[mt][i].w};
#pragma unroll
                for (int nt = 0; nt < 4; ++nt) u0[nt] = __builtin_amdgcn_mfma_f32_16x16x4f32(t[nt], p0[mt][i], u0[nt], 0, 0, 0);
            }
        }
    };
    auto softmax = [&](f32x4 (&lg)[NMT], const int4 (&ids)[NMT]) {
        float mx = -INFINITY;
#pragma unroll
        for (int mt = 0; mt < NMT; ++mt) {
            const int id[4] = {ids[mt].x, ids[mt].y, ids[mt].z, ids[mt].w};
#pragma unroll
            for (int i = 0; i < 4; ++i) mx = fmaxf(mx, id[i] >= 0 ? lg[mt][i] : -INFINITY);
        }
        mx = xor32_max(xor16_max(mx));
        float z = 0.f;
#pragma unroll
        for (int mt = 0; mt < NMT; ++mt) {
            const int id[4] = {ids[mt].x, ids[mt].y, ids[mt].z, ids[mt].w};
#pragma unroll
            for (int i = 0; i < 4; ++i) {
                const float x = lean_exp(fminf(lg[mt][i] - mx, 0.f));
                const float e = id[i] >= 0 ? x : 0.f;
                lg[mt][i] = e;
                z += e;
            }
        }
        z = xor32_sum(xor16_sum(z));
        const float inv = 1.f / z;
#pragma unroll
        for (int mt = 0; mt < NMT; ++mt) {
#pragma unroll
            for (int i = 0; i < 4; ++i) lg[mt][i] *= inv;
        }
    };

    int iter = 0;
    auto stamp = [&](int slot) {
        if constexpr (TRACE) {
            if (blockIdx.x == 0 && threadIdx.x == 0 && iter >= 2 && iter < 66) g_kaf_trace[(iter - 2) * 16 + slot] = __builtin_readcyclecounter();
        }
    };
    auto load_item_raw = [&](const int (&orig)[2], unsigned (&item)[2]) {
#pragma unroll
        for (int rt = 0; rt < 2; ++rt)
            item[rt] = a.items64 ? reinterpret_cast<const unsigned*>(a.items64)[2 * (int64_t)orig[rt]] : (unsigned)a.items32[orig[rt]];
    };
    auto load_item = [&](const int (&orig)[2], unsigned (&item)[2]) {
        load_item_raw(orig, item);
#pragma unroll
        for (int rt = 0; rt < 2; ++rt) item[rt] = min(item[rt], emax);
    };

    const int wave = __builtin_amdgcn_readfirstlane((int)(threadIdx.x >> 6));
    const int stride = (int)gridDim.x * kFlashWaves;
    const int recW = (1 + 2 * P) * NmP, ldsT = NmP, ldsHr = NmP + P * NmP;
    const unsigned lds0 = (unsigned)(size_t)(__attribute__((address_space(3))) char*)sKafRec + (unsigned)(wave * 2 * recW * 4);
    const int lorig = kFlashWaves * 2 * recW + wave * 32;
    const unsigned ldsOrig = (unsigned)(size_t)(__attribute__((address_space(3))) char*)sKafRec + (unsigned)(lorig * 4);
    auto la_slots_issue = [&](long long base) -> int {
        const long long kc = base + (long long)stride * (lane + 1);
        return kc < a.nslots ? a.slot_seg[kc] : -1;
    };
    auto la_slots_take = [&](long long base, int sv, int& kN, int& sN) -> bool {
        for (;;) {
            const unsigned long long live = __ballot(sv >= 0);
            if (live) {
                const int j = __ffsll(live) - 1;
                kN = __builtin_amdgcn_readfirstlane((int)(base + (long long)stride * (j + 1)));
                sN = __builtin_amdgcn_readlane(sv, j);
                return true;
            }
            base += 64ll * stride;
            if (base + stride >= a.nslots) return false;
            sv = la_slots_issue(base);
        }
    };
    auto la_seg_issue = [&](int s) -> int {
        const int32_t* src = lane == 0 ? a.seg_user + s : a.seg_ptr + s + (lane - 1);
        return lane < 3 ? *src : 0;
    };
    auto la_seg_take = [&](int v, int k, int s, int& u, int& cbeg, int& cend) {
        u = __builtin_amdgcn_readlane(v, 0);
        const int p0 = __builtin_amdgcn_readlane(v, 1), p1 = __builtin_amdgcn_readlane(v, 2);
        cbeg = p0 + (k - (p0 / kFlashChunk + s)) * kFlashChunk;
        cend = min(p1, cbeg + kFlashChunk);
    };
    auto la_rec_issue = [&](int u, int cbeg, int cend, int par) {
        const char* src = reinterpret_cast<const char*>(a.records + (size_t)u * RL.len);
        const unsigned dst = lds0 + (unsigned)(par * recW * 4);
        for (int j0 = 0; j0 < recW; j0 += 64) {
// ... 171 lines not shown
            if constexpr (!PF) load_item(orig, item);
#pragma unroll
            for (int mt = 0; mt < NMT; ++mt) issue_u(mt, hrC, R);
            if constexpr (PF) laSlots = la_slots_issue(k);
        }
        load_be(item, bE);
        if constexpr (PF && !HAS_SET) {
            KAF_FENCE();
            la_step_slots();
        }
#pragma unroll
        for (int nt = 0; nt < 4; ++nt) myUo0[nt][lane] = uo0[nt];
        KAF_FENCE();
        stamp(2);

        const int ntile = (cend - cbeg + 31) >> 5;
        int t0 = cbeg;
        int stage = 0;
        const int stage_items = min(2, 2 * ntile * P - 1);
        auto la_stage = [&]() {
            if constexpr (PF) {
                if (stage == 0) la_step_seg();
                if (stage == stage_items) la_step_items(stage_items == 2);
                ++stage;
                KAF_FENCE();
            }
        };
        auto run_tile = [&](const bool two, const bool more) {
            f32x4 uo[2][4];
#pragma unroll
            for (int rt = 0; rt < 2; ++rt) {
#pragma unroll
                for (int nt = 0; nt < 4; ++nt) uo[rt][nt] = myUo0[nt][lane];
            }
            unsigned itemN[2];
            if (more) load_item(origN, itemN);
            for (int hop = 0; hop < P; ++hop) {
                const bool last_hop = hop + 1 == P;
                const bool next_stage = !last_hop || more;
                const int hopN = last_hop ? 0 : hop + 1;
                const float* __restrict__ tw = a.TW + (size_t)(hop + (HAS_SET ? 1 : 0)) * tw_stride;
                if (next_stage) load_hr(hopN, hrN);
                KAF_FENCE();
                if (t0 == cbeg && hop < 3) stamp(3 + 4 * hop);
                f32x4 lg[2][NMT];
#pragma unroll
                for (int mt = 0; mt < NMT; ++mt) {
                    lg[0][mt] = f32x4{0.f, 0.f, 0.f, 0.f};
                    lg[1][mt] = f32x4{0.f, 0.f, 0.f, 0.f};
                    if (two) {
#pragma unroll
                        for (int nt = 0; nt < 4; ++nt) {
                            const float av[4] = {R.v[mt][nt].x, R.v[mt][nt].y, R.v[mt][nt].z, R.v[mt][nt].w};
                            const float e0[4] = {bE[0][nt].x, bE[0][nt].y, bE[0][nt].z, bE[0][nt].w};
                            const float e1[4] = {bE[1][nt].x, bE[1][nt].y, bE[1][nt].z, bE[1][nt].w};
#pragma unroll
                            for (int i = 0; i < 4; ++i) {
                                lg[0][mt] = __builtin_amdgcn_mfma_f32_16x16x4f32(av[i], e0[i], lg[0][mt], 0, 0, 0);
                                lg[1][mt] = __builtin_amdgcn_mfma_f32_16x16x4f32(av[i], e1[i], lg[1][mt], 0, 0, 0);
                            }
                        }
                    } else {
#pragma unroll
                        for (int nt = 0; nt < 4; ++nt) {
                            const float av[4] = {R.v[mt][nt].x, R.v[mt][nt].y, R.v[mt][nt].z, R.v[mt][nt].w};
                            const float e0[4] = {bE[0][nt].x, bE[0][nt].y, bE[0][nt].z, bE[0][nt].w};
#pragma unroll
                            for (int i = 0; i < 4; ++i) lg[0][mt] = __builtin_amdgcn_mfma_f32_16x16x4f32(av[i], e0[i], lg[0][mt], 0, 0, 0);
                        }
                    }
                    KAF_FENCE();
                    issue_t(mt, tw, tidC, R);
                    KAF_FENCE();
                }
                if (last_hop && more) load_be(itemN, bE);
                KAF_FENCE();
                if (t0 == cbeg && hop < 3) stamp(4 + 4 * hop);
                la_stage();
                softmax(lg[0], tidC);
                if (two) softmax(lg[1], tidC);
                KAF_FENCE();
                if (t0 == cbeg && hop < 3) stamp(5 + 4 * hop);
#pragma unroll
                for (int mt = 0; mt < NMT; ++mt) {
                    reads_tile(two, mt, R, lg[0], lg[1], uo[0], uo[1]);
                    KAF_FENCE();
                    if (next_stage) issue_u(mt, hrN, R);
                    KAF_FENCE();
                }
                if (next_stage) load_tid(hopN, tidC);
                if (t0 == cbeg && hop < 3) stamp(6 + 4 * hop);
                la_stage();
            }
#pragma unroll
            for (int rt = 0; rt < 2; ++rt) {
                if (valid[rt] && (rt == 0 || two)) {
#pragma unroll
                    for (int r = 0; r < 4; ++r)
                        *reinterpret_cast<float4*>(a.user_o + (size_t)orig[rt] * D + 16 * q16 + 4 * r) =
                            make_float4(uo[rt][0][r], uo[rt][1][r], uo[rt][2][r], uo[rt][3][r]);
                }
            }
        };
        for (int tile = 0; tile < ntile; ++tile, t0 += 32) {
            const bool more = tile + 1 < ntile;
            run_tile(cend - t0 > 16, more);
#pragma unroll
            for (int rt = 0; rt < 2; ++rt) orig[rt] = origN[rt], valid[rt] = validN[rt];
        }
        stamp(15);
        par ^= 1;
    }
}

hipError_t kaf_read_trace(long long* host_dst, size_t n) {
    const size_t have = sizeof(g_kaf_trace) / sizeof(long long);
    return hipMemcpyFromSymbol(host_dst, HIP_SYMBOL(g_kaf_trace), (n < have ? n : have) * sizeof(long long));
}
#undef KAF_FENCE

bool key_addr_flash_supported(int D, int P, int Nm, int nR, int n_entity) {
    if (D != 64 || P < 1 || P > 8 || Nm < 1 || Nm > 64) return false;
    const KaRecLayout RL = ka_rec_layout(P, Nm, nR);
    if (RL.len == 0) return false;
    return (long long)nR * n_entity < (1ll << 31);
}

size_t key_addr_flash_ws_elems(int64_t B, int nseg_bound) { return (size_t)(B / kFlashChunk + nseg_bound + 1) + 1; }

static int env_int(const char* name, int dflt) {
    const char* v = getenv(name);
    return v && *v ? atoi(v) : dflt;
}

template <int NMT>
static hipError_t launch_flash_n(const KaFlashArgs& a, const KaRecLayout& RL, bool has_set, hipStream_t st) {
    static const bool prefetch = env_int("MVIN_KAF_PREFETCH", 1) != 0;
    static const int grid_cap = env_int("MVIN_KAF_GRID", 0);
    auto k = prefetch ? (has_set ? key_addr_flash_kernel<NMT, true, true> : key_addr_flash_kernel<NMT, false, true>)
                      : (has_set ? key_addr_flash_kernel<NMT, true, false> : key_addr_flash_kernel<NMT, false, false>);
    if constexpr (NMT == 4) {
        static const bool trace = getenv("MVIN_KAF_TRACE") != nullptr;
        if (trace && has_set) k = prefetch ? key_addr_flash_kernel<4, true, true, true> : key_addr_flash_kernel<4, true, false, true>;
    }
    const size_t lds = prefetch ? (size_t)kFlashWaves * (2 * (1 + 2 * a.P) * RL.NmP + 32) * sizeof(int32_t) : 0;
    const int pc = workgroups_per_cu(k, kFlashWaves * 64, lds, 2);
    const int64_t want = ((int64_t)a.nslots + kFlashWaves - 1) / kFlashWaves;
    int grid = (int)persistent_grid(want, pc > 8 ? 8 : pc);
    if (grid_cap > 0 && grid > grid_cap) grid = grid_cap;
    k<<<grid, kFlashWaves * 64, lds, st>>>(a, RL);
    return hipGetLastError();
}

hipError_t launch_key_addr_flash(const KaFlashArgs& a_, int nseg_bound, bool has_set, int32_t* sched_ws, hipStream_t st) {
    KaFlashArgs a = a_;
    const KaRecLayout RL = ka_rec_layout(a.P, a.Nm, a.nR);
    if (RL.len == 0 || !sched_ws) return hipErrorInvalidValue;
    if (!a.bmlp) {
        void* zeros = nullptr;
        if (hipError_t e = hipGetSymbolAddress(&zeros, HIP_SYMBOL(g_kaf_no_bias)); e != hipSuccess) return e;
        a.bmlp = static_cast<const float*>(zeros);
    }
    a.nslots = (int)(a.B / kFlashChunk + nseg_bound + 1);
    a.slot_seg = sched_ws;
    a.counter = sched_ws + a.nslots;
    hipError_t e = hipMemsetAsync(sched_ws, 0xFF, ((size_t)a.nslots + 1) * sizeof(int32_t), st);
    if (e != hipSuccess) return e;
    {
        const int blocks = nseg_bound < 256 * 64 ? (nseg_bound + 255) / 256 : 64;
        ka_flash_slots_kernel<<<blocks > 0 ? blocks : 1, 256, 0, st>>>(a.seg_ptr, a.nseg_dev, nseg_bound, sched_ws);
        e = hipGetLastError();
        if (e != hipSuccess) return e;
    }
    switch (RL.NmP / 16) {
        case 1: return launch_flash_n<1>(a, RL, has_set, st);
        case 2: return launch_flash_n<2>(a, RL, has_set, st);
        case 3: return launch_flash_n<3>(a, RL, has_set, st);
        case 4: return launch_flash_n<4>(a, RL, has_set, st);
        default: return hipErrorInvalidValue;
    }
}

}
```

### mvin_amd/csrc/mvin_keyaddr_static.hip

```cpp
#include <cstdlib>
#include <utility>

#include "mvin_kernels.h"

namespace mvin {

typedef float f32x4 __attribute__((ext_vector_type(4)));

__device__ __forceinline__ float kas_exp(float x) {
    const float t = x * 1.44269502162933349609375f;
    const float n = rintf(t);
    float f = fmaf(x, 1.44269502162933349609375f, -n);
    f = fmaf(x, 1.925963033500011e-8f, f);
    return ldexpf(__builtin_amdgcn_exp2f(f), (int)n);
}

__device__ long long g_kas_trace[64 * 16];

constexpr int kSW = 12;
constexpr int kSSide = 4;
constexpr int kRT = 2;
constexpr int kST = 16 * kRT;
constexpr int kSMaxRows = 128;

__host__ __device__ constexpr int kas_pad4(int v) { return (v + 3) & ~3; }
__host__ __device__ constexpr KaRecLayout ka_rec_layout_c(int P, int Nm, int nR) {
    KaRecLayout R{};
    if (P < 1 || P > 8 || Nm < 1 || Nm > 256 || nR < 1 || nR > 4096) return R;
    R.NmP = (Nm + 15) & ~15;
    R.rows = P * R.NmP;
    const int nrl = nR < P * Nm ? nR : P * Nm;
    R.maxtiles = R.rows / 16 + nrl;
    R.o_cnt = 4;
    R.o_off = R.o_cnt + kas_pad4(nR);
    R.o_trel = R.o_off + kas_pad4(nR);
    R.o_bidx = R.o_trel + kas_pad4(R.maxtiles);
    R.o_head = R.o_bidx + R.maxtiles * 16;
    R.o_tail = R.o_head + R.rows;
    R.o_hr = R.o_tail + R.rows;
    R.len = (R.o_hr + R.rows + 63) & ~63;
    return R;
}
KaRecLayout ka_rec_layout(int P, int Nm, int nR) { return ka_rec_layout_c(P, Nm, nR); }

__global__ __launch_bounds__(64) void user_records_kernel(const int32_t* __restrict__ uts, int n_user, int P, int Nm, int nR, int n_entity,
                                                           KaRecLayout RL, int32_t* __restrict__ out) {
    extern __shared__ int s_rec[];
    int* sCnt = s_rec;
    int* sOff = s_rec + nR;
    const int u = blockIdx.x, lane = threadIdx.x;
    if (u >= n_user) return;
    int32_t* rec = out + (size_t)u * RL.len;
    const int32_t* ub = uts + (int64_t)u * P * 3 * Nm;
    const unsigned emax = (unsigned)(n_entity - 1);
    if (lane >= 1 && lane < 4) rec[lane] = 0;
    for (int r = lane; r < nR; r += 64) sCnt[r] = 0;
    __syncthreads();
    auto row_rel = [&](int i) -> int {
        const int hop = i / RL.NmP, m = i - hop * RL.NmP;
        if (i >= RL.rows || m >= Nm) return -1;
        return (int)min((unsigned)ub[(hop * 3 + 1) * Nm + m], (unsigned)(nR - 1));
    };
    for (int i0 = 0; i0 < RL.rows; i0 += 64) {
        const int r = row_rel(i0 + lane);
        if (r >= 0) atomicAdd(&sCnt[r], 1);
    }
    __syncthreads();
    int ntile = 0;
    for (int r0 = 0; r0 < nR; r0 += 64) {
        const int r = r0 + lane;
        const int cnt = r < nR ? sCnt[r] : 0;
        const int tiles = (cnt + 15) >> 4;
        int incl = tiles;
#pragma unroll
        for (int o = 1; o < 64; o <<= 1) {
            const int v = __shfl_up(incl, o, 64);
            if (lane >= o) incl += v;
        }
        const int first = ntile + incl - tiles;
        if (r < nR) {
            rec[RL.o_cnt + r] = cnt;
            rec[RL.o_off + r] = first * 16;
            sOff[r] = first * 16;
            for (int j = 0; j < tiles; ++j) rec[RL.o_trel + first + j] = r;
        }
        ntile += __shfl(incl, 63, 64);
    }
    if (lane == 0) rec[0] = ntile;
    __syncthreads();
    for (int r = lane; r < nR; r += 64) sCnt[r] = 0;
    __syncthreads();
    for (int i0 = 0; i0 < RL.rows; i0 += 64) {
        const int i = i0 + lane;
        const int r = row_rel(i);
        int before = 0;
        bool last = true;
        for (int l = 0; l < 64; ++l) {
            const int rl = __shfl(r, l, 64);
            if (rl == r && l < lane) ++before;
            if (rl == r && l > lane) last = false;
        }
        if (r >= 0) {
            const int at = sCnt[r] + before;
            rec[RL.o_bidx + sOff[r] + at] = i;
            const int hop = i / RL.NmP, m = i - hop * RL.NmP;
            const int hd = (int)min((unsigned)ub[(hop * 3 + 0) * Nm + m], emax);
            rec[RL.o_head + i] = hd;
            rec[RL.o_tail + i] = (int)min((unsigned)ub[(hop * 3 + 2) * Nm + m], emax);
            const long long hr = (long long)r * n_entity + hd;
            rec[RL.o_hr + i] = hr < (1ll << 31) ? (int)hr : 0;
        }
        __syncthreads();
        if (r >= 0 && last) sCnt[r] += before + 1;
        __syncthreads();
    }
}

hipError_t launch_user_records(const int32_t* uts, int n_user, int P, int Nm, int nR, int n_entity, int32_t* out, hipStream_t st) {
    const KaRecLayout RL = ka_rec_layout(P, Nm, nR);
    if (RL.len == 0) return hipErrorInvalidValue;
    hipError_t e = hipMemsetAsync(out, 0xFF, (size_t)n_user * RL.len * sizeof(int32_t), st);
    if (e != hipSuccess) return e;
    user_records_kernel<<<n_user, 64, (size_t)2 * nR * sizeof(int), st>>>(uts, n_user, P, Nm, nR, n_entity, RL, out);
    return hipGetLastError();
}

struct KaStaticLds {
    int h, u, t, ei, l, z, hset, rec, orig, desc, total;
};

__host__ __device__ constexpr KaStaticLds ka_static_layout(int P, const KaRecLayout& RL) {
    KaStaticLds L{};
    constexpr int D = 64;
    int o = 0;
    auto take = [&](int words) { const int at = o; o += (words + 3) & ~3; return at; };
    L.rec = take(2 * RL.len);
    L.h = take(RL.rows * (D + 4));
    L.u = take((RL.rows + 1) * (D + 4));
    L.t = take(RL.rows * D);
    L.ei = take(2 * kST * (D + 4));
    L.l = take(kST * (RL.rows + 2));
    L.z = take(kST * P);
    L.hset = take(D);
    L.orig = take(2 * kST);
    L.desc = take(4);
    L.total = o * 4;
    return L;
}

template <int J>
__device__ __forceinline__ void kas_dma_line(const char* p, int lane4, int n) {
    if (J < n) asm volatile("global_load_lds_dword %0, %1 offset:%2" ::"v"(lane4), "s"(p), "n"(J * 256) : "memory");
}
template <int... J>
__device__ __forceinline__ void kas_dma_lines(const char* p, int lane4, unsigned m0, int n, std::integer_sequence<int, J...>) {
// ... 432 lines not shown
                    }
#pragma unroll
                    for (int rt = 0; rt < kRT; ++rt) {
                        if (rt < nrt) {
#pragma unroll
                            for (int i = 0; i < 4; ++i) sL[(size_t)(16 * rt + 4 * KAS_Q16 + i) * LDL + 16 * mt + KAS_L16] = acc[rt][i];
                        }
                    }
                }
            }
            if (t0 == p0) stamp(10);
            __syncthreads();
            relane();
            if (t0 == p0) stamp(6);
            if (side) {
                chain_b();
                if (heads) {
                    stage_write(stg, recn + RL.o_head, sj * 2 * kHalf, sH, LDH, false);
                    stage_issue(stg, recn + RL.o_head, sj * 2 * kHalf + kHalf);
                }
            } else {
                const int rg = lane >> 4, cl = lane & 15;
                for (int base = wave * 4; base < 16 * nrt * P; base += kMW * 4) {
                    const int task = base + rg;
                    const bool ok = task < 16 * nrt * P;
                    const int tk = ok ? task : base;
                    const int pi = tk / P, hop = tk - pi * P;
                    float* row = sL + (size_t)pi * LDL + hop * NmP;
                    float mx = -INFINITY, z = 0.f;
                    if (NmP <= 64) {
                        float v[4];
#pragma unroll
                        for (int u = 0; u < 4; ++u) v[u] = (cl + 16 * u < Nm) ? row[cl + 16 * u] : -INFINITY;
                        mx = group_max(fmaxf(fmaxf(v[0], v[1]), fmaxf(v[2], v[3])), 4);
#pragma unroll
                        for (int u = 0; u < 4; ++u) {
                            const float e = (cl + 16 * u < Nm) ? kas_exp(v[u] - mx) : 0.f;
                            if (ok && cl + 16 * u < NmP) row[cl + 16 * u] = e;
                            z += e;
                        }
                    } else {
                        for (int m = cl; m < Nm; m += 16) mx = fmaxf(mx, row[m]);
                        mx = group_max(mx, 4);
                        for (int m = cl; m < NmP; m += 16) {
                            const float e = m < Nm ? kas_exp(row[m] - mx) : 0.f;
                            if (ok) row[m] = e;
                            z += e;
                        }
                    }
                    z = group_sum(z, 4);
                    if (ok && cl == 0) sZ[task] = 1.f / z;
                }
            }
            if (t0 == p0) stamp(11);
            __syncthreads();
            relane();
            if (t0 == p0) stamp(7);
            if (side) {
                if (heads) stage_write(stg, recn + RL.o_head, sj * 2 * kHalf + kHalf, sH, LDH, false);
                chain_c(ep ^ 1);
            } else {
                for (int task = wave; task < P * NT; task += kMW) {
                    const int hop = task / NT, nt = task - hop * NT;
                    f32x4 acc[kRT];
#pragma unroll
                    for (int rt = 0; rt < kRT; ++rt) acc[rt] = f32x4{0.f, 0.f, 0.f, 0.f};
                    const float* ar = sL + (size_t)KAS_L16 * LDL + hop * NmP + KAS_Q16;
                    const float* br = sT + (size_t)(hop * NmP + KAS_Q16) * LDT + 16 * (nt ^ KAS_Q16) + KAS_L16;
                    if (nrt == kRT) {
                        for (int k = 0; k < NmP / 4; k += 4) {
                            float av[kRT][4], bv[4];
#pragma unroll
                            for (int u = 0; u < 4; ++u) {
                                bv[u] = br[(size_t)4 * (k + u) * LDT];
#pragma unroll
                                for (int rt = 0; rt < kRT; ++rt) av[rt][u] = ar[(size_t)16 * rt * LDL + 4 * (k + u)];
                            }
#pragma unroll
                            for (int u = 0; u < 4; ++u) {
#pragma unroll
                                for (int rt = 0; rt < kRT; ++rt) acc[rt] = __builtin_amdgcn_mfma_f32_16x16x4f32(av[rt][u], bv[u], acc[rt], 0, 0, 0);
                            }
                        }
                    } else {
                        for (int k = 0; k < NmP / 4; k += 4) {
                            float av[4], bv[4];
#pragma unroll
                            for (int u = 0; u < 4; ++u) {
                                av[u] = ar[4 * (k + u)];
                                bv[u] = br[(size_t)4 * (k + u) * LDT];
                            }
#pragma unroll
                            for (int u = 0; u < 4; ++u) acc[0] = __builtin_amdgcn_mfma_f32_16x16x4f32(av[u], bv[u], acc[0], 0, 0, 0);
                        }
                    }
#pragma unroll
                    for (int rt = 0; rt < kRT; ++rt) {
                        if (rt < nrt) {
#pragma unroll
                            for (int i = 0; i < 4; ++i) {
                                const int pi = 16 * rt + 4 * KAS_Q16 + i;
                                const int orig = sOc[pi];
                                if (orig >= 0)
                                    a.out[(size_t)((unsigned)orig * ldo32 + (unsigned)((slot0 + hop) * D + 16 * nt + KAS_L16))] = acc[rt][i] * sZ[pi * P + hop];
                            }
                        }
                    }
                }
                if (has_set) {
                    for (int i = KAS_TID; i < 16 * nrt * LPR; i += kMW * 64) {
                        const int pi = i / LPR, cc = i - pi * LPR;
                        const int orig = sOc[pi];
                        if (orig >= 0)
                            *reinterpret_cast<float4*>(a.out + (size_t)((unsigned)orig * ldo32 + (unsigned)(4 * cc))) = *reinterpret_cast<const float4*>(sHset + 4 * cc);
                    }
                }
            }
            if (t0 == p0) stamp(8);
        }
        if (p0 >= p1) {
            __syncthreads();
            rotate();
            if (has_next) heads_now(recn);
            chain_a(p00, p10);
            chain_b();
            chain_c(ep);
        }
    }
}
#undef KAS_Q16
#undef KAS_L16
#undef KAS_TID
#undef KAS_ITID

bool key_addr_static_supported(int D, int P, int Nm, int nR) {
    if (D != 64) return false;
    const KaRecLayout RL = ka_rec_layout(P, Nm, nR);
    if (RL.len == 0 || RL.rows < 64 || RL.rows > kSMaxRows) return false;
    return ka_static_layout(P, RL).total <= 160 * 1024;
}

bool key_addr_static_applies(const KeyAddrGroupedArgs& a, int table_bf16) {
    static const bool off = getenv("MVIN_KA_STATIC") && atoi(getenv("MVIN_KA_STATIC")) == 0;
    return !off && a.records != nullptr && !table_bf16 && key_addr_static_supported(a.D, a.P, a.Nm, a.nR) &&
           (int64_t)a.nseg * a.ldo < (int64_t(1) << 31);
}

bool key_addr_static_er_ok(int P, int Nm, int nR, int n_entity, bool has_set) {
    const KaRecLayout RL = ka_rec_layout(P, Nm, nR);
    return RL.len != 0 && (!has_set || RL.NmP <= 64) && (long long)nR * n_entity < (1ll << 31);
}

__global__ __launch_bounds__(256) void entity_dot_kernel(const float* __restrict__ E, const float* __restrict__ w, int n, int D, float* __restrict__ out) {
    const int lane = threadIdx.x & 63, g = lane >> 4, c = lane & 15;
    const int64_t row = ((int64_t)blockIdx.x * 4 + (threadIdx.x >> 6)) * 4 + g;
    float s = 0.f;
    if (row < n)
        for (int d = 4 * c; d < D; d += 64) {
            const float4 e4 = *reinterpret_cast<const float4*>(E + row * D + d), w4 = *reinterpret_cast<const float4*>(w + d);
            s = fmaf(e4.x, w4.x, fmaf(e4.y, w4.y, fmaf(e4.z, w4.z, fmaf(e4.w, w4.w, s))));
        }
    s = group_sum(s, 4);
    if (row < n && c == 0) out[row] = s;
}

__global__ void transpose_blocks_kernel(const float* __restrict__ R, int D, float* __restrict__ RT) {
    const int r = blockIdx.x / D, k = blockIdx.x % D, n = threadIdx.x;
    if (n < D) RT[((size_t)r * D + k) * D + n] = R[((size_t)r * D + n) * D + k];
}

hipError_t launch_transpose_blocks(const float* R, int nR, int D, float* RT, hipStream_t st) {
    transpose_blocks_kernel<<<nR * D, D < 64 ? 64 : D, 0, st>>>(R, D, RT);
    return hipGetLastError();
}

hipError_t launch_entity_dot(const float* E, const float* w, int n, int D, float* out, hipStream_t st) {
    entity_dot_kernel<<<(n + 15) / 16, 256, 0, st>>>(E, w, n, D, out);
    return hipGetLastError();
}

hipError_t kas_read_trace(long long* host_dst, size_t n) {
    const size_t have = sizeof(g_kas_trace) / sizeof(long long);
    return hipMemcpyFromSymbol(host_dst, HIP_SYMBOL(g_kas_trace), (n < have ? n : have) * sizeof(long long));
}

hipError_t launch_key_addr_static(const KeyAddrGroupedArgs& a, hipStream_t st) {
    const KaRecLayout RL = ka_rec_layout(a.P, a.Nm, a.nR);
    const KaStaticLds L = ka_static_layout(a.P, RL);
    static const bool trace = getenv("MVIN_KA_TRACE") != nullptr;
    const bool c3 = a.P == 2 && a.Nm == 64 && a.nR == 9 && !(getenv("MVIN_KAS_GENERIC") && atoi(getenv("MVIN_KAS_GENERIC")));
    const bool er = a.ER != nullptr;
    auto k = er ? (c3 ? (trace ? key_addr_static_kernel<true, 2, 64, 9, true> : key_addr_static_kernel<false, 2, 64, 9, true>)
                      : key_addr_static_kernel<false, 0, 0, 0, true>)
                : c3 ? (trace ? key_addr_static_kernel<true, 2, 64, 9> : key_addr_static_kernel<false, 2, 64, 9>)
                     : (trace ? key_addr_static_kernel<true, 0, 0, 0> : key_addr_static_kernel<false, 0, 0, 0>);
    if (hipError_t e = grant_lds(k, L.total); e != hipSuccess) return e;
    KeyAddrGroupedArgs b = a;
    b.dbg = 0;
    if (trace) {
        const char* tw = getenv("MVIN_KA_TRACE_WAVE");
        b.dbg = tw ? atoi(tw) % kSW : 0;
    }
    const int grid = (int)persistent_grid(a.nseg, 1);
    k<<<grid, kSW * 64, L.total, st>>>(b, RL, L);
    return hipGetLastError();
}

}
```

### mvin_amd/csrc/mvin_workspaces.h

```cpp
#pragma once
#include <cstddef>
#include <cstdint>

#ifdef __HIPCC__
#define MVIN_WS_FN __host__ __device__ constexpr
#else
#define MVIN_WS_FN constexpr
#endif

namespace mvin {

struct FoldBlock {
    size_t D, DD;
    MVIN_WS_FN explicit FoldBlock(int d) : D((size_t)d), DD((size_t)d * (size_t)d) {}
    MVIN_WS_FN size_t Wstack(int i = 0) const { return (size_t)i * DD; }
    MVIN_WS_FN size_t Wv() const { return Wstack(4); }
    MVIN_WS_FN size_t Wq() const { return Wv() + DD; }
    MVIN_WS_FN size_t bv() const { return Wq() + DD; }
    MVIN_WS_FN size_t bq() const { return bv() + D; }
    MVIN_WS_FN size_t bm() const { return bq() + D; }
    MVIN_WS_FN size_t Wperm(int k = 0) const { return bm() + D + (size_t)k * DD; }
    MVIN_WS_FN size_t elems() const { return Wperm(6); }
};

struct FoldWs {
    size_t tab;
    FoldBlock blk;
    MVIN_WS_FN FoldWs(int n_entity, int D) : tab((size_t)n_entity * (size_t)D), blk(D) {}
    MVIN_WS_FN size_t table(int i) const { return (size_t)i * tab; }
    MVIN_WS_FN size_t TA1() const { return table(0); }
    MVIN_WS_FN size_t TA2() const { return table(1); }
    MVIN_WS_FN size_t T0A() const { return table(2); }
    MVIN_WS_FN size_t M0() const { return table(3); }
    MVIN_WS_FN size_t H0() const { return table(4); }
    MVIN_WS_FN size_t G() const { return table(5); }
    MVIN_WS_FN size_t block() const { return table(6); }
    MVIN_WS_FN size_t elems() const { return block() + blk.elems(); }
};

struct PrjBlock {
    size_t D, DD;
    MVIN_WS_FN explicit PrjBlock(int d) : D((size_t)d), DD((size_t)d * (size_t)d) {}
    MVIN_WS_FN size_t Wstack(int i = 0) const { return (size_t)i * DD; }
    MVIN_WS_FN size_t Wv() const { return Wstack(3); }
    MVIN_WS_FN size_t b1c() const { return Wv() + DD; }
    MVIN_WS_FN size_t bv() const { return b1c() + D; }
    MVIN_WS_FN size_t elems() const { return bv() + D; }
};

struct PrjWs {
    size_t tab;
    PrjBlock blk;
    MVIN_WS_FN PrjWs(int n_entity, int D) : tab((size_t)n_entity * (size_t)D), blk(D) {}
    MVIN_WS_FN size_t table(int i) const { return (size_t)i * tab; }
    MVIN_WS_FN size_t T1() const { return table(0); }
    MVIN_WS_FN size_t TA1() const { return table(1); }
    MVIN_WS_FN size_t TA2() const { return table(2); }
    MVIN_WS_FN size_t block() const { return table(3); }
    MVIN_WS_FN size_t elems() const { return block() + blk.elems(); }
};

struct AggWs {
    size_t tab;
    MVIN_WS_FN AggWs(int n_entity, int D) : tab((size_t)n_entity * (size_t)D) {}
    MVIN_WS_FN size_t S0() const { return 0; }
    MVIN_WS_FN size_t G() const { return tab; }
    MVIN_WS_FN size_t elems() const { return G() + tab; }
};

struct RelWs {
    size_t tab, n_entity, nR, DD;
    MVIN_WS_FN RelWs(int n_entity_, int nR_, int D) : tab((size_t)n_entity_ * (size_t)D), n_entity((size_t)n_entity_), nR((size_t)nR_), DD((size_t)D * (size_t)D) {}
    MVIN_WS_FN size_t ER(int r = 0) const { return (size_t)r * tab; }
    MVIN_WS_FN size_t hs() const { return nR * tab; }
    MVIN_WS_FN size_t RT() const { return hs() + ((n_entity + 3) & ~(size_t)3); }
    MVIN_WS_FN size_t elems() const { return RT() + nR * DD; }
    MVIN_WS_FN size_t TW(int j = 0) const { return elems() + (size_t)j * tab; }
    MVIN_WS_FN size_t flash_elems(int n_o) const { return TW(n_o); }
};

struct GroupWs {
    size_t n_user, B;
    MVIN_WS_FN GroupWs(int n_user_, int64_t B_) : n_user((size_t)n_user_), B((size_t)B_) {}
    MVIN_WS_FN size_t counters() const { return 0; }
    MVIN_WS_FN size_t offsets() const { return n_user; }
    MVIN_WS_FN size_t ranks() const { return offsets() + n_user; }
    MVIN_WS_FN size_t sort_elems() const { return ranks() + B; }
    MVIN_WS_FN size_t seg_user() const { return sort_elems(); }
    MVIN_WS_FN size_t seg_ptr() const { return seg_user() + B; }
    MVIN_WS_FN size_t nseg() const { return seg_ptr() + B + 2; }
    MVIN_WS_FN size_t pair_index() const { return nseg() + 1; }
    MVIN_WS_FN size_t elems() const { return pair_index() + B; }
    MVIN_WS_FN size_t flash_sched() const { return counters(); }
    MVIN_WS_FN bool flash_sched_fits(size_t need) const { return need <= sort_elems(); }
};

}
```

Before: 585.0 million.

## Fuse step prologue kernel and build flash slots inside group scan

Adds a single step-prologue kernel that folds the weight block preparation, the entity·w dot product and the clearing of the per-user counters into one launch, and lets the group scan kernel write the flash schedule slots directly into unused group workspace. This skips the separate fold prepare, the entity_dot launch, the counter memset, the slot memset and the slot-building kernel on the flash path. The aim is to cut launch count and small serialized kernels in the scoring step. The path is gated by an env var and shape and alignment checks, and it adds workspace aliasing that must not overlap live data.

```diff
diff --git a/mvin_amd/build.py b/mvin_amd/build.py
--- a/mvin_amd/build.py
+++ b/mvin_amd/build.py
@@ -13,7 +13,7 @@
 OBJ_DIR = os.path.join(PKG_DIR, "_build")
 SOURCES = ["mvin_kernels.hip", "mvin_fused.hip", "mvin_fused_split.hip", "mvin_fused_packed.hip", "mvin_fused_wpp.hip", "mvin_fused_agg.hip", "mvin_fused_agg32.hip", "mvin_fused_wpp_fold.hip", "mvin_fused_d16.hip", "mvin_fused_d32.hip", "mvin_tail.hip", "mvin_tail_flash.hip", "mvin_score_small.hip", "mvin_keyaddr.hip", "mvin_keyaddr_stream.hip", "mvin_keyaddr_grouped.hip", "mvin_keyaddr_dense.hip", "mvin_keyaddr_static.hip", "mvin_keyaddr_flash.hip", "mvin_keyaddr_wave.hip", "mvin_hoist.hip", "mvin_probe.hip", "mvin_group.hip", "mvin_order.hip", "mvin_topk.hip", "mvin_rank.hip", "mvin_segments.hip", "mvin_mmr.hip", "mvin_mips.hip", "mvin_resample.hip", "mvin_explore.hip", "mvin_ctr_metrics.hip", "mvin_ctr_delong.hip", "mvin_ctr_curve.hip", "mvin_ctr_rank_resample.hip","mvin_ctr_cluster.hip", "mvin_ctr_segments.hip", "mvin_ctr_calib.hip", "mvin_rank_head.hip", "mvin_mf.hip", "mvin_select_negatives.hip", "mvin_explain.hip", "mvin_explain_mem.hip", "mvin_prep.hip", "mvin_negatives.hip", "mvin_linear_mfma.hip", "mvin_entity_tables.hip", "mvin_bwd.hip", "mvin_grad_guard.hip",
            "mvin_abi_basic.hip", "mvin_abi_levels.hip", "mvin_abi_keyaddr.hip", "mvin_abi_score.hip", "mvin_abi_eval.hip", "mvin_abi_train.hip"]
-HEADERS = ["mvin_common.h", "mvin_kernels.h", "mvin_launch.h", "mvin_fused_agg.h", "mvin_score_image.h", "mvin_ctr_bodies.h", "mvin_row_select.h", "mvin_rnd.h", "mvin_explain_mass.h", "mvin_rank_head_body.h",
+HEADERS = ["mvin_common.h", "mvin_entity_dot.h", "mvin_kernels.h", "mvin_launch.h", "mvin_fused_agg.h", "mvin_score_image.h", "mvin_ctr_bodies.h", "mvin_row_select.h", "mvin_rnd.h", "mvin_explain_mass.h", "mvin_rank_head_body.h",
            "mvin_workspaces.h", "mvin_score_plan.h", "mvin_abi_util.h", "mvin_entity_tables_plan.h", "mvin_l2_kernel_plan.h"]
 VERSION_SCRIPT = os.path.join(CSRC, "libmvin_hip.map")
 ARCH = "gfx950"
diff --git a/mvin_amd/csrc/mvin_abi_keyaddr.hip b/mvin_amd/csrc/mvin_abi_keyaddr.hip
--- a/mvin_amd/csrc/mvin_abi_keyaddr.hip
+++ b/mvin_amd/csrc/mvin_abi_keyaddr.hip
@@ -5,7 +5,7 @@
 
 int group_pairs_impl(const int64_t* users_i64, const int32_t* users_i32, int64_t B, int n_user, int32_t* workspace, int32_t* seg_user,
                      int32_t* seg_ptr, int32_t* nseg, int32_t* pair_index, void* stream, const int64_t* items64, unsigned max_id,
-                     int32_t* item_rows) {
+                     int32_t* item_rows, const GroupStepFront* front) {
     const char* who = "mvin_group_pairs_by_user";
     if ((!users_i64 && !users_i32) || !workspace || !seg_user || !seg_ptr || !nseg || !pair_index)
         return fail(-1, "%s: null pointer", who);
@@ -13,19 +13,57 @@
     const GroupWs L(n_user, B);
     return hip_result(mvin::launch_group_pairs(users_i64, users_i32, B, n_user, workspace + L.counters(), workspace + L.offsets(),
                                                workspace + L.ranks(), seg_user, seg_ptr, nseg, pair_index, (hipStream_t)stream,
-                                               reinterpret_cast<const int32_t*>(items64), 2, max_id, item_rows), who);
+                                               reinterpret_cast<const int32_t*>(items64), 2, max_id, item_rows, front), who);
 }
 
 int flash_prepare_impl(const char* who, const float* entity_emb, const float* relation_kge, const float* w, const float* user_mlp_W, int n_entity,
-                       int nR, int D, int P, float* ws, float* fold_ws, void* stream) {
+                       int nR, int D, int P, float* ws, float* fold_ws, void* stream, bool hs_written) {
     if (!entity_emb || !relation_kge || !user_mlp_W || !ws) return fail(-1, "%s: null pointer", who);
     if (n_entity <= 0 || nR <= 0 || D != 64 || P < 1 || P > 8) return fail(-2, "%s: n_entity=%d nR=%d D=%d P=%d", who, n_entity, nR, D, P);
     const RelWs L(n_entity, nR, D);
     if (int rc = build_entity_tables(who, entity_emb, n_entity, relation_kge, nR, ws + L.ER(), user_mlp_W, P + (w ? 1 : 0), ws + L.TW(),
                                      fold_ws ? fold_ws + FoldWs(n_entity, D).block() : nullptr, fold_ws, stream))
         return rc;
-    if (w) return hip_result(mvin::launch_entity_dot(entity_emb, w, n_entity, D, ws + L.hs(), (hipStream_t)stream), who);
+    if (w && !hs_written) return hip_result(mvin::launch_entity_dot(entity_emb, w, n_entity, D, ws + L.hs(), (hipStream_t)stream), who);
     return 0;
+}
+
+static int flash_nseg_bound(int64_t B, int n_user) { return (int)(B < (int64_t)n_user ? B : (int64_t)n_user); }
+
+int flash_fwd_impl(const float* entity_emb, const float* ws, const int32_t* user_records, const int32_t* seg_user, const int32_t* seg_ptr,
+                   const int32_t* nseg_dev, const int32_t* pair_index, const int64_t* items_i64, const int32_t* items_i32, int64_t B, int P, int Nm,
+                   int D, int nR, int n_entity, int n_user, int has_set, const float* user_mlp_b, float* user_o, int32_t* sched_ws, void* stream,
+                   bool slots_built) {
+    const char* who = "mvin_key_addressing_flash_fwd";
+    if (!entity_emb || !ws || !user_records || !seg_user || !seg_ptr || !pair_index || !user_o || !sched_ws)
+        return fail(-1, "%s: null pointer", who);
+    if ((items_i64 == nullptr) == (items_i32 == nullptr)) return fail(-1, "%s: exactly one of items_i64 / items_i32", who);
+    if (B <= 0 || B >= (int64_t(1) << 31) || n_user <= 0 || n_entity <= 0 || nR <= 0)
+        return fail(-2, "%s: bad sizes B=%lld n_user=%d n_entity=%d nR=%d", who, (long long)B, n_user, n_entity, nR);
+    if (!mvin::key_addr_flash_supported(D, P, Nm, nR, n_entity))
+        return fail(-3, "%s: unsupported shape D=%d P=%d Nm=%d nR=%d n_entity=%d (D = 64, 1 <= P <= 8, Nm <= 64, nR * n_entity < 2^31)", who,
+                    D, P, Nm, nR, n_entity);
+    mvin::KaFlashArgs k{};
+    k.E = entity_emb;
+    const mvin::RelWs L(n_entity, nR, D);
+    k.ER = ws + L.ER();
+    k.hs = has_set ? ws + L.hs() : nullptr;
+    k.TW = ws + L.TW();
+    k.records = user_records;
+    k.seg_user = seg_user;
+    k.seg_ptr = seg_ptr;
+    k.nseg_dev = nseg_dev;
+    k.pair_index = pair_index;
+    k.items64 = items_i64;
+    k.items32 = items_i32;
+    k.bmlp = user_mlp_b;
+    k.user_o = user_o;
+    k.P = P;
+    k.Nm = Nm;
+    k.nR = nR;
+    k.n_entity = n_entity;
+    k.B = B;
+    return hip_result(mvin::launch_key_addr_flash(k, flash_nseg_bound(B, n_user), has_set != 0, sched_ws, (hipStream_t)stream, slots_built), who);
 }
 
 }
@@ -174,8 +212,6 @@
     return mvin::key_addr_flash_supported(D, P, Nm, nR, n_entity) ? 1 : 0;
 }
 
-static int flash_nseg_bound(int64_t B, int n_user) { return (int)(B < (int64_t)n_user ? B : (int64_t)n_user); }
-
 size_t mvin_key_addressing_flash_ws_elems(int64_t B, int n_user) {
     if (B <= 0 || n_user <= 0) return 0;
     return mvin::key_addr_flash_ws_elems(B, flash_nseg_bound(B, n_user));
@@ -196,36 +232,8 @@
                                   const int32_t* seg_ptr, const int32_t* nseg_dev, const int32_t* pair_index, const int64_t* items_i64,
                                   const int32_t* items_i32, int64_t B, int P, int Nm, int D, int nR, int n_entity, int n_user, int has_set,
                                   const float* user_mlp_b, float* user_o, int32_t* sched_ws, void* stream) {
-    const char* who = "mvin_key_addressing_flash_fwd";
-    if (!entity_emb || !ws || !user_records || !seg_user || !seg_ptr || !pair_index || !user_o || !sched_ws)
-        return fail(-1, "%s: null pointer", who);
-    if ((items_i64 == nullptr) == (items_i32 == nullptr)) return fail(-1, "%s: exactly one of items_i64 / items_i32", who);
-    if (B <= 0 || B >= (int64_t(1) << 31) || n_user <= 0 || n_entity <= 0 || nR <= 0)
-        return fail(-2, "%s: bad sizes B=%lld n_user=%d n_entity=%d nR=%d", who, (long long)B, n_user, n_entity, nR);
-    if (!mvin::key_addr_flash_supported(D, P, Nm, nR, n_entity))
-        return fail(-3, "%s: unsupported shape D=%d P=%d Nm=%d nR=%d n_entity=%d (D = 64, 1 <= P <= 8, Nm <= 64, nR * n_entity < 2^31)", who,
-                    D, P, Nm, nR, n_entity);
-    mvin::KaFlashArgs k{};
-    k.E = entity_emb;
-    const mvin::RelWs L(n_entity, nR, D);
-    k.ER = ws + L.ER();
-    k.hs = has_set ? ws + L.hs() : nullptr;
-    k.TW = ws + L.TW();
-    k.records = user_records;
-    k.seg_user = seg_user;
-    k.seg_ptr = seg_ptr;
-    k.nseg_dev = nseg_dev;
-    k.pair_index = pair_index;
-    k.items64 = items_i64;
-    k.items32 = items_i32;
-    k.bmlp = user_mlp_b;
-    k.user_o = user_o;
-    k.P = P;
-    k.Nm = Nm;
-    k.nR = nR;
-    k.n_entity = n_entity;
-    k.B = B;
-    return hip_result(mvin::launch_key_addr_flash(k, flash_nseg_bound(B, n_user), has_set != 0, sched_ws, (hipStream_t)stream), who);
+    return flash_fwd_impl(entity_emb, ws, user_records, seg_user, seg_ptr, nseg_dev, pair_index, items_i64, items_i32, B, P, Nm, D, nR, n_entity,
+                          n_user, has_set, user_mlp_b, user_o, sched_ws, stream, false);
 }
 
 static int key_addressing_grouped_impl(const void* entity_emb, const float* relation_kge, const float* w,
diff --git a/mvin_amd/csrc/mvin_abi_score.hip b/mvin_amd/csrc/mvin_abi_score.hip
--- a/mvin_amd/csrc/mvin_abi_score.hip
+++ b/mvin_amd/csrc/mvin_abi_score.hip
@@ -33,6 +33,12 @@
     return in;
 }
 
+bool step_front_form(const mvin_score_l2_args* a, const mvin::ScorePlan& plan, const mvin::StepPrologueArgs& pro) {
+    static const bool on = !(getenv("MVIN_STEP_FRONT") && atoi(getenv("MVIN_STEP_FRONT")) == 0);
+    return on && plan.ka == KeyAddrForm::Flash && plan.fold_in_flash && a->D == 64 && a->h_set_w && !mvin::group_pairs_small(a->B, a->n_user) &&
+           mvin::GroupWs(a->n_user, a->B).scan_sched_fits(mvin_key_addressing_flash_ws_elems(a->B, a->n_user)) && mvin::step_prologue_aligned(pro);
+}
+
 int project_v(const mvin_score_l2_args* a, void* stream) {
     const int D = a->D, nR = a->n_relation;
     mvin_linear_args l{};
@@ -106,10 +112,32 @@
 
     const mvin::GroupWs G(a->n_user, a->B);
     int32_t* const gws = a->group_ws;
+    mvin::StepPrologueArgs pro{};
+    pro.W0 = a->W0, pro.b0 = a->b0, pro.W1 = a->W1, pro.b1 = a->b1, pro.W2 = a->W2, pro.b2 = a->b2, pro.A0 = a->A0, pro.a0 = a->a0;
+    pro.Wmix = a->Wmix, pro.bmix = a->bmix, pro.A1 = a->A1, pro.E = E, pro.w = a->h_set_w, pro.n_entity = nE, pro.n_user = a->n_user;
+    const bool front = step_front_form(a, plan, pro);
+    mvin::GroupStepFront gfront{};
+    if (front) {
+        rc = fold_tables_check("mvin_fold_tables", E, a->enc_entity, a->enc_relation, a->W0, a->W1, a->W2, a->A0, a->Wmix, a->A1,
+                               plan.deep == DeepForm::Folded, K, D, nE, nR, a->fold_ws);
+        if (rc) return rc;
+        if (!a->relation_kge || !a->user_mlp_W || !a->ka_flash) return fail(-1, "%s: null pointer", "mvin_key_addressing_flash_prepare");
+        pro.c = a->t0 ? 1.f / (float)K : 1.f;
+        pro.blk = a->fold_ws + mvin::FoldWs(nE, D).block();
+        pro.hs = a->ka_flash + mvin::RelWs(nE, nR, D).hs();
+        pro.count = gws + G.counters();
+        rc = hip_result(mvin::launch_step_prologue(pro, (hipStream_t)stream), who);
+        if (rc) return rc;
+        gfront.counters_clear = true;
+        gfront.slot_seg = gws + G.scan_sched();
+        gfront.nslots = (int)mvin_key_addressing_flash_ws_elems(a->B, a->n_user) - 1;
+    }
+
     int32_t *seg_user = nullptr, *seg_ptr = nullptr, *nseg = nullptr, *pair_index = nullptr;
     if (plan.grouped()) {
         seg_user = gws + G.seg_user(), seg_ptr = gws + G.seg_ptr(), nseg = gws + G.nseg(), pair_index = gws + G.pair_index();
-        rc = group_pairs_impl(a->users, nullptr, a->B, a->n_user, gws, seg_user, seg_ptr, nseg, pair_index, stream, a->items, item_max, item_rows);
+        rc = group_pairs_impl(a->users, nullptr, a->B, a->n_user, gws, seg_user, seg_ptr, nseg, pair_index, stream, a->items, item_max, item_rows,
+                              front ? &gfront : nullptr);
         if (rc) return rc;
     }
     if (plan.project_v) {
@@ -119,7 +147,7 @@
 
     switch (plan.ka) {
         case KeyAddrForm::Flash:
-            if (plan.fold_in_flash) {
+            if (plan.fold_in_flash && !front) {
                 rc = fold_tables_check("mvin_fold_tables", E, a->enc_entity, a->enc_relation, a->W0, a->W1, a->W2, a->A0, a->Wmix, a->A1,
                                        plan.deep == DeepForm::Folded, K, D, nE, nR, a->fold_ws);
                 if (rc) return rc;
@@ -128,13 +156,13 @@
                 if (rc) return rc;
             }
             rc = flash_prepare_impl("mvin_key_addressing_flash_prepare", E, a->relation_kge, a->h_set_w, a->user_mlp_W, nE, nR, D, a->P,
-                                    a->ka_flash, plan.fold_in_flash ? a->fold_ws : nullptr, stream);
-            if (rc) return rc;
-            if (!G.flash_sched_fits(mvin_key_addressing_flash_ws_elems(a->B, a->n_user)))
+                                    a->ka_flash, plan.fold_in_flash ? a->fold_ws : nullptr, stream, front);
+            if (rc) return rc;
+            if (!front && !G.flash_sched_fits(mvin_key_addressing_flash_ws_elems(a->B, a->n_user)))
                 return fail(-2, "%s: group_ws too small for the flash form's scheduling scratch", who);
-            rc = mvin_key_addressing_flash_fwd(E, a->ka_flash, a->user_records, seg_user, seg_ptr, nseg, pair_index, a->items, nullptr, a->B,
-                                               a->P, a->Nm, D, nR, nE, a->n_user, a->h_set_w != nullptr, a->user_mlp_b, a->user_o,
-                                               gws + G.flash_sched(), stream);
+            rc = flash_fwd_impl(E, a->ka_flash, a->user_records, seg_user, seg_ptr, nseg, pair_index, a->items, nullptr, a->B, a->P, a->Nm, D, nR,
+                                nE, a->n_user, a->h_set_w != nullptr, a->user_mlp_b, a->user_o, gws + (front ? G.scan_sched() : G.flash_sched()),
+                                stream, front);
             break;
         case KeyAddrForm::GatheredER:
             rc = mvin_project_relations(E, a->relation_kge, a->h_set_w, nE, nR, D, a->ka_er, stream);
diff --git a/mvin_amd/csrc/mvin_abi_util.h b/mvin_amd/csrc/mvin_abi_util.h
--- a/mvin_amd/csrc/mvin_abi_util.h
+++ b/mvin_amd/csrc/mvin_abi_util.h
@@ -54,10 +54,14 @@
                      void* stream, const int32_t* rows_s);
 
 int flash_prepare_impl(const char* who, const float* entity_emb, const float* relation_kge, const float* w, const float* user_mlp_W, int n_entity,
-                       int nR, int D, int P, float* ws, float* fold_ws, void* stream);
+                       int nR, int D, int P, float* ws, float* fold_ws, void* stream, bool hs_written = false);
 int group_pairs_impl(const int64_t* users_i64, const int32_t* users_i32, int64_t B, int n_user, int32_t* workspace, int32_t* seg_user,
                      int32_t* seg_ptr, int32_t* nseg, int32_t* pair_index, void* stream, const int64_t* items64, unsigned max_id,
-                     int32_t* item_rows);
+                     int32_t* item_rows, const GroupStepFront* front = nullptr);
+int flash_fwd_impl(const float* entity_emb, const float* ws, const int32_t* user_records, const int32_t* seg_user, const int32_t* seg_ptr,
+                   const int32_t* nseg_dev, const int32_t* pair_index, const int64_t* items_i64, const int32_t* items_i32, int64_t B, int P, int Nm,
+                   int D, int nR, int n_entity, int n_user, int has_set, const float* user_mlp_b, float* user_o, int32_t* sched_ws, void* stream,
+                   bool slots_built);
 
 }
 }
diff --git a/mvin_amd/csrc/mvin_entity_dot.h b/mvin_amd/csrc/mvin_entity_dot.h
--- /dev/null
+++ b/mvin_amd/csrc/mvin_entity_dot.h
@@ -0,0 +1,30 @@
+#pragma once
+#include "mvin_common.h"
+
+namespace mvin {
+
+template <int UN>
+__device__ __forceinline__ void entity_dot_rows(const float* __restrict__ E, const float* __restrict__ w, int n, int D, float* __restrict__ out,
+                                                int64_t unit) {
+    const int lane = threadIdx.x & 63, g = lane >> 4, c = lane & 15;
+    const int64_t row0 = ((unit * 4 + (threadIdx.x >> 6)) * UN) * 4 + g;
+    float s[UN];
+#pragma unroll
+    for (int u = 0; u < UN; ++u) s[u] = 0.f;
+    for (int d = 4 * c; d < D; d += 64) {
+        const float4 w4 = *reinterpret_cast<const float4*>(w + d);
+        float4 e4[UN];
+#pragma unroll
+        for (int u = 0; u < UN; ++u)
+            e4[u] = row0 + 4 * u < n ? *reinterpret_cast<const float4*>(E + (row0 + 4 * u) * D + d) : make_float4(0.f, 0.f, 0.f, 0.f);
+#pragma unroll
+        for (int u = 0; u < UN; ++u) s[u] = fmaf(e4[u].x, w4.x, fmaf(e4[u].y, w4.y, fmaf(e4[u].z, w4.z, fmaf(e4[u].w, w4.w, s[u]))));
+    }
+#pragma unroll
+    for (int u = 0; u < UN; ++u) {
+        s[u] = group_sum(s[u], 4);
+        if (row0 + 4 * u < n && c == 0) out[row0 + 4 * u] = s[u];
+    }
+}
+
+}
diff --git a/mvin_amd/csrc/mvin_fused_agg.hip b/mvin_amd/csrc/mvin_fused_agg.hip
--- a/mvin_amd/csrc/mvin_fused_agg.hip
+++ b/mvin_amd/csrc/mvin_fused_agg.hip
@@ -1,3 +1,4 @@
+#include "mvin_entity_dot.h"
 #include "mvin_fused_agg.h"
 #include "mvin_workspaces.h"
 
@@ -770,26 +771,38 @@
     }
 }
 
-__global__ void fold_prepare_kernel(const float* __restrict__ W0, const float* __restrict__ b0, const float* __restrict__ W1,
-                                    const float* __restrict__ b1, const float* __restrict__ W2, const float* __restrict__ b2,
-                                    const float* __restrict__ A0, const float* __restrict__ a0, const float* __restrict__ Wmix,
-                                    const float* __restrict__ bmix, const float* __restrict__ A1, float c, int D, float* __restrict__ blk) {
-    const int i = blockIdx.x, j = threadIdx.x;
+struct FoldSrcGlobal {
+    const float *__restrict__ W0, *__restrict__ b0, *__restrict__ W1, *__restrict__ b1, *__restrict__ W2, *__restrict__ b2, *__restrict__ A0,
+        *__restrict__ a0, *__restrict__ Wmix, *__restrict__ bmix, *__restrict__ A1;
+    int i, j, D;
+    __device__ float av(int k) const { return A0[(size_t)k * D + j]; }
+    __device__ float mv(int k) const { return Wmix[(size_t)k * D + j]; }
+    __device__ float x0(int k) const { return i < D ? W0[(size_t)i * D + k] : (b0 ? b0[k] : 0.f); }
+    __device__ float x1(int k) const { return i < D ? W1[(size_t)i * D + k] : (b1 ? b1[k] : 0.f); }
+    __device__ float x2(int k) const { return i < D ? W2[(size_t)i * D + k] : (b2 ? b2[k] : 0.f); }
+    __device__ float a1_ij() const { return A1[(size_t)i * D + j]; }
+    __device__ float wm1_ij() const { return Wmix[(size_t)D * D + (size_t)i * D + j]; }
+    __device__ float wm2_ij() const { return Wmix[2 * (size_t)D * D + (size_t)i * D + j]; }
+    __device__ float a0_j() const { return a0 ? a0[j] : 0.f; }
+    __device__ float bmix_j() const { return bmix ? bmix[j] : 0.f; }
+};
+
+template <int KR, class Src>
+__device__ __forceinline__ void fold_prepare_row(const Src& src, int i, int j, int D, float c, float* __restrict__ blk) {
     const FoldBlock L(D);
-    if (j >= D) return;
     float s0 = 0.f, s1 = 0.f, s2 = 0.f, sm = 0.f;
-    for (int k0 = 0; k0 < D; k0 += 8) {
-        float av[8], mv[8], x0[8], x1[8], x2[8];
-#pragma unroll
-        for (int k = 0; k < 8; ++k) {
-            av[k] = A0[(size_t)(k0 + k) * D + j];
-            mv[k] = Wmix[(size_t)(k0 + k) * D + j];
-            x0[k] = i < D ? W0[(size_t)i * D + k0 + k] : (b0 ? b0[k0 + k] : 0.f);
-            x1[k] = i < D ? W1[(size_t)i * D + k0 + k] : (b1 ? b1[k0 + k] : 0.f);
-            x2[k] = i < D ? W2[(size_t)i * D + k0 + k] : (b2 ? b2[k0 + k] : 0.f);
-        }
-#pragma unroll
-        for (int k = 0; k < 8; ++k) {
+    for (int k0 = 0; k0 < D; k0 += KR) {
+        float av[KR], mv[KR], x0[KR], x1[KR], x2[KR];
+#pragma unroll
+        for (int k = 0; k < KR; ++k) {
+            av[k] = src.av(k0 + k);
+            mv[k] = src.mv(k0 + k);
+            x0[k] = src.x0(k0 + k);
+            x1[k] = src.x1(k0 + k);
+            x2[k] = src.x2(k0 + k);
+        }
+#pragma unroll
+        for (int k = 0; k < KR; ++k) {
             s0 = fmaf(x0[k], av[k], s0);
             s1 = fmaf(x1[k], av[k], s1);
             s2 = fmaf(x2[k], av[k], s2);
@@ -809,21 +822,104 @@
             blk[L.Wperm(0) + o] = fmaf(c, s1, s0);
             blk[L.Wperm(1) + o] = fmaf(c, s2, s1);
             blk[L.Wperm(2) + o] = sm;
-            blk[L.Wperm(3) + o] = A1[ij];
-            blk[L.Wperm(4) + o] = Wmix[L.DD + ij];
-            blk[L.Wperm(5) + o] = Wmix[2 * L.DD + ij];
+            blk[L.Wperm(3) + o] = src.a1_ij();
+            blk[L.Wperm(4) + o] = src.wm1_ij();
+            blk[L.Wperm(5) + o] = src.wm2_ij();
         }
     } else {
-        const float av0 = a0 ? a0[j] : 0.f;
+        const float av0 = src.a0_j();
         blk[L.bv() + j] = fmaf(c, s2, s1) + av0;
         blk[L.bq() + j] = fmaf(c, s1, s0) + av0;
-        blk[L.bm() + j] = (bmix ? bmix[j] : 0.f) + sm;
-    }
+        blk[L.bm() + j] = src.bmix_j() + sm;
+    }
+}
+
+__global__ void fold_prepare_kernel(const float* __restrict__ W0, const float* __restrict__ b0, const float* __restrict__ W1,
+                                    const float* __restrict__ b1, const float* __restrict__ W2, const float* __restrict__ b2,
+                                    const float* __restrict__ A0, const float* __restrict__ a0, const float* __restrict__ Wmix,
+                                    const float* __restrict__ bmix, const float* __restrict__ A1, float c, int D, float* __restrict__ blk) {
+    const int i = blockIdx.x, j = threadIdx.x;
+    if (j >= D) return;
+    fold_prepare_row<8>(FoldSrcGlobal{W0, b0, W1, b1, W2, b2, A0, a0, Wmix, bmix, A1, i, j, D}, i, j, D, c, blk);
 }
 
 hipError_t launch_fold_prepare(const float* W0, const float* b0, const float* W1, const float* b1, const float* W2, const float* b2, const float* A0,
                                const float* a0, const float* Wmix, const float* bmix, const float* A1, float c, int D, float* blk, hipStream_t st) {
     fold_prepare_kernel<<<D + 1, D < 64 ? 64 : D, 0, st>>>(W0, b0, W1, b1, W2, b2, A0, a0, Wmix, bmix, A1, c, D, blk);
+    return hipGetLastError();
+}
+
+struct FoldSrcStaged {
+    const float *sA, *sM, *sX;
+    float t0, t1, t2;
+    int j;
+    __device__ float av(int k) const { return sA[k * 64 + j]; }
+    __device__ float mv(int k) const { return sM[k * 64 + j]; }
+    __device__ float x0(int k) const { return sX[k]; }
+    __device__ float x1(int k) const { return sX[64 + k]; }
+    __device__ float x2(int k) const { return sX[128 + k]; }
+    __device__ float a1_ij() const { return t0; }
+    __device__ float wm1_ij() const { return t1; }
+    __device__ float wm2_ij() const { return t2; }
+    __device__ float a0_j() const { return t0; }
+    __device__ float bmix_j() const { return t1; }
+};
+
+constexpr int kPrologueRows = 4;
+constexpr int kPrologueClear = 2048;
+constexpr int kPrologueDotUN = 4;
+
+__global__ __launch_bounds__(256) void step_prologue_kernel(StepPrologueArgs a) {
+    constexpr int D = 64;
+    __shared__ __attribute__((aligned(16))) float sA[D * D], sM[D * D], sX[kPrologueRows][3][D];
+    const int tid = threadIdx.x;
+    int b = blockIdx.x;
+    if (b < a.na) {
+        const int wave = tid >> 6, j = tid & 63, i = kPrologueRows * b + wave;
+        float4 a4[4], m4[4];
+#pragma unroll
+        for (int q = 0; q < 4; ++q) {
+            a4[q] = reinterpret_cast<const float4*>(a.A0)[q * 256 + tid];
+            m4[q] = reinterpret_cast<const float4*>(a.Wmix)[q * 256 + tid];
+        }
+        float x[3] = {0.f, 0.f, 0.f}, t[3] = {0.f, 0.f, 0.f};
+        if (i < D) {
+            const int ij = i * D + j;
+            x[0] = a.W0[ij], x[1] = a.W1[ij], x[2] = a.W2[ij];
+            t[0] = a.A1[ij], t[1] = a.Wmix[D * D + ij], t[2] = a.Wmix[2 * D * D + ij];
+        } else if (i == D) {
+            x[0] = a.b0 ? a.b0[j] : 0.f, x[1] = a.b1 ? a.b1[j] : 0.f, x[2] = a.b2 ? a.b2[j] : 0.f;
+            t[0] = a.a0 ? a.a0[j] : 0.f, t[1] = a.bmix ? a.bmix[j] : 0.f;
+        }
+#pragma unroll
+        for (int q = 0; q < 4; ++q) {
+            reinterpret_cast<float4*>(sA)[q * 256 + tid] = a4[q];
+            reinterpret_cast<float4*>(sM)[q * 256 + tid] = m4[q];
+        }
+#pragma unroll
+        for (int m = 0; m < 3; ++m) sX[wave][m][j] = x[m];
+        __syncthreads();
+        if (i <= D) fold_prepare_row<16>(FoldSrcStaged{sA, sM, &sX[wave][0][0], t[0], t[1], t[2], j}, i, j, D, a.c, a.blk);
+        return;
+    }
+    b -= a.na;
+    if (b < a.nc) {
+#pragma unroll
+        for (int q = 0; q < kPrologueClear / 256; ++q) {
+            const int u = b * kPrologueClear + q * 256 + tid;
+            if (u < a.n_user) a.count[u] = 0;
+        }
+        return;
+    }
+    entity_dot_rows<kPrologueDotUN>(a.E, a.w, a.n_entity, D, a.hs, b - a.nc);
+}
+
+hipError_t launch_step_prologue(const StepPrologueArgs& a_, hipStream_t st) {
+    StepPrologueArgs a = a_;
+    a.na = (64 + 1 + kPrologueRows - 1) / kPrologueRows;
+    a.nc = (a.n_user + kPrologueClear - 1) / kPrologueClear;
+    const int nb = (a.n_entity + 16 * kPrologueDotUN - 1) / (16 * kPrologueDotUN);
+    step_prologue_kernel<<<a.na + a.nc + nb, 256, 0, st>>>(a);
     return hipGetLastError();
 }
 
diff --git a/mvin_amd/csrc/mvin_group.hip b/mvin_amd/csrc/mvin_group.hip
--- a/mvin_amd/csrc/mvin_group.hip
+++ b/mvin_amd/csrc/mvin_group.hip
@@ -93,7 +93,7 @@
                                                           int32_t* __restrict__ offs, int32_t* __restrict__ seg_user,
                                                           int32_t* __restrict__ seg_ptr, int32_t* __restrict__ nseg,
                                                           const int32_t* __restrict__ block_rows, int nblocks,
-                                                          int32_t* __restrict__ item_rows) {
+                                                          int32_t* __restrict__ item_rows, int32_t* __restrict__ slot_seg, int nslots) {
     extern __shared__ int sCnt[];
     int* sSeg = sCnt + min(n_user, kScanTile);
     __shared__ int sC[16], sS[16], sRows[16];
@@ -145,9 +145,17 @@
             if (sg >= 0) {
                 seg_user[sg] = t0 + u;
                 seg_ptr[sg] = o;
+                if (slot_seg) {
+                    const int p1 = u + 1 < n ? sCnt[u + 1] : carryC;
+                    const int first = o / kFlashChunk + sg, live = first + (p1 - o + kFlashChunk - 1) / kFlashChunk;
+                    const int next = min(p1 / kFlashChunk + sg + 1, nslots);
+                    for (int k = first; k < next; ++k) slot_seg[k] = k < live ? sg : -1;
+                }
             }
         }
     }
+    if (slot_seg)
+        for (int k = carryC / kFlashChunk + carryS + tid; k <= nslots; k += 1024) slot_seg[k] = -1;
     if (tid == 0) {
         nseg[0] = carryS;
         seg_ptr[carryS] = carryC;
@@ -244,19 +252,25 @@
 constexpr int64_t kGroupSmallMaxB = 32768;
 constexpr size_t kGroupSmallMaxLds = 150 * 1024;
 
+bool group_pairs_small(int64_t B, int n_user) {
+    static const int force = getenv("MVIN_GROUP_SMALL") ? atoi(getenv("MVIN_GROUP_SMALL")) : -1;
+    return (size_t)n_user * sizeof(int32_t) <= kGroupSmallMaxLds && (force < 0 ? B <= kGroupSmallMaxB : force == 1);
+}
+
 hipError_t launch_group_pairs(const int64_t* u64, const int32_t* u32, int64_t B, int n_user, int32_t* count, int32_t* offs,
                               int32_t* rank, int32_t* seg_user, int32_t* seg_ptr, int32_t* nseg, int32_t* pair_index, hipStream_t st,
-                              const int32_t* items, int item_stride, unsigned max_id, int32_t* item_rows) {
+                              const int32_t* items, int item_stride, unsigned max_id, int32_t* item_rows, const GroupStepFront* front) {
     if (!items) item_rows = nullptr;
-    static const int force = getenv("MVIN_GROUP_SMALL") ? atoi(getenv("MVIN_GROUP_SMALL")) : -1;
     const size_t lds = (size_t)n_user * sizeof(int32_t);
-    const bool small = lds <= kGroupSmallMaxLds && (force < 0 ? B <= kGroupSmallMaxB : force == 1);
+    const bool small = group_pairs_small(B, n_user);
     if (small) {
+        if (front) return hipErrorInvalidValue;
         if (hipError_t e = grant_lds(group_small_kernel, lds, 48 * 1024); e != hipSuccess) return e;
         group_small_kernel<<<1, 1024, lds, st>>>(u64, u32, B, n_user, seg_user, seg_ptr, nseg, pair_index, items, item_stride, max_id, item_rows);
         return hipGetLastError();
     }
-    hipError_t e = hipMemsetAsync(count, 0, (size_t)n_user * sizeof(int32_t), st);
+    hipError_t e = hipSuccess;
+    if (!(front && front->counters_clear)) e = hipMemsetAsync(count, 0, (size_t)n_user * sizeof(int32_t), st);
     if (e != hipSuccess) return e;
     const int blocks = (int)((B + 255) / 256 < 2048 ? (B + 255) / 256 : 2048);
     group_count_kernel<<<blocks, 256, 0, st>>>(u64, u32, B, n_user, count, rank, items, item_stride, max_id, item_rows ? pair_index : nullptr);
@@ -264,7 +278,8 @@
         const size_t scan_lds = (size_t)2 * (n_user < kScanTile ? n_user : kScanTile) * sizeof(int32_t);
         e = grant_lds(group_scan_kernel, scan_lds, 48 * 1024);
         if (e != hipSuccess) return e;
-        group_scan_kernel<<<1, 1024, scan_lds, st>>>(count, n_user, B, offs, seg_user, seg_ptr, nseg, pair_index, blocks, item_rows);
+        group_scan_kernel<<<1, 1024, scan_lds, st>>>(count, n_user, B, offs, seg_user, seg_ptr, nseg, pair_index, blocks, item_rows,
+                                                     front ? front->slot_seg : nullptr, front ? front->nslots : 0);
     }
     group_scatter_kernel<<<blocks, 256, 0, st>>>(u64, u32, B, n_user, offs, rank, pair_index);
     return hipGetLastError();
diff --git a/mvin_amd/csrc/mvin_kernels.h b/mvin_amd/csrc/mvin_kernels.h
--- a/mvin_amd/csrc/mvin_kernels.h
+++ b/mvin_amd/csrc/mvin_kernels.h
@@ -367,8 +367,9 @@
 bool key_addr_static_applies(const KeyAddrGroupedArgs& a, int table_bf16);
 hipError_t launch_key_addr_static(const KeyAddrGroupedArgs& a, hipStream_t st);
 bool key_addr_flash_supported(int D, int P, int Nm, int nR, int n_entity);
+constexpr int kFlashChunk = 64;
 size_t key_addr_flash_ws_elems(int64_t B, int nseg_bound);
-hipError_t launch_key_addr_flash(const KaFlashArgs& a, int nseg_bound, bool has_set, int32_t* sched_ws, hipStream_t st);
+hipError_t launch_key_addr_flash(const KaFlashArgs& a, int nseg_bound, bool has_set, int32_t* sched_ws, hipStream_t st, bool slots_built = false);
 hipError_t kas_read_trace(long long* host_dst, size_t n);
 hipError_t kaf_read_trace(long long* host_dst, size_t n);
 hipError_t fold_read_trace(long long* host_dst, size_t n);
@@ -424,9 +425,16 @@
 hipError_t launch_gather_attn_l2(const FusedL2Args& a, int D, int table_bf16, hipStream_t st);
 hipError_t launch_gather_probe_l2(const void* table, const int32_t* ids1, const int32_t* ids2, int64_t n_parents, int K,
                                   int D, int table_bf16, float* sums, hipStream_t st);
+struct GroupStepFront {
+    bool counters_clear;
+    int32_t* slot_seg;
+    int nslots;
+};
+bool group_pairs_small(int64_t B, int n_user);
 hipError_t launch_group_pairs(const int64_t* u64, const int32_t* u32, int64_t B, int n_user, int32_t* count, int32_t* offs,
                               int32_t* rank, int32_t* seg_user, int32_t* seg_ptr, int32_t* nseg, int32_t* pair_index, hipStream_t st,
-                              const int32_t* items = nullptr, int item_stride = 1, unsigned max_id = 0, int32_t* item_rows = nullptr);
+                              const int32_t* items = nullptr, int item_stride = 1, unsigned max_id = 0, int32_t* item_rows = nullptr,
+                              const GroupStepFront* front = nullptr);
 hipError_t launch_item_rows(const int32_t* items, int item_stride, int64_t B, unsigned max_id, int32_t* item_rows, hipStream_t st);
 hipError_t launch_count_ids(const int32_t* ids, int64_t n, int nbins, float* out, hipStream_t st);
 bool topk_rows_supported(int k);
@@ -575,6 +583,21 @@
 hipError_t launch_entity_aggregates(const EntityAggArgs& a, hipStream_t st);
 hipError_t launch_fold_prepare(const float* W0, const float* b0, const float* W1, const float* b1, const float* W2, const float* b2, const float* A0,
                                const float* a0, const float* Wmix, const float* bmix, const float* A1, float c, int D, float* blk, hipStream_t st);
+struct StepPrologueArgs {
+    const float *W0, *b0, *W1, *b1, *W2, *b2, *A0, *a0, *Wmix, *bmix, *A1;
+    float c;
+    float* blk;
+    const float *E, *w;
+    int n_entity;
+    float* hs;
+    int32_t* count;
+    int n_user;
+    int na, nc;
+};
+inline bool step_prologue_aligned(const StepPrologueArgs& a) {
+    return ((reinterpret_cast<uintptr_t>(a.A0) | reinterpret_cast<uintptr_t>(a.Wmix) | reinterpret_cast<uintptr_t>(a.E) | reinterpret_cast<uintptr_t>(a.w)) & 15) == 0;
+}
+hipError_t launch_step_prologue(const StepPrologueArgs& a, hipStream_t st);
 hipError_t launch_l2_tail_fold(const TailFoldArgs& a, hipStream_t st);
 hipError_t launch_score_l2_folded(const float* agg, const float* M0, const int32_t* adj_e, const int32_t* adj_r, const int32_t* items, int pid_stride,
                                   const float* t1, const float* q, const float* user_o, const float* Wq, const float* bq, const float* Wv,
diff --git a/mvin_amd/csrc/mvin_keyaddr_flash.hip b/mvin_amd/csrc/mvin_keyaddr_flash.hip
--- a/mvin_amd/csrc/mvin_keyaddr_flash.hip
+++ b/mvin_amd/csrc/mvin_keyaddr_flash.hip
@@ -7,7 +7,6 @@
 
 typedef float f32x4 __attribute__((ext_vector_type(4)));
 
-constexpr int kFlashChunk = 64;
 constexpr int kFlashWaves = 4;
 
 __global__ void ka_flash_slots_kernel(const int32_t* __restrict__ seg_ptr, const int32_t* __restrict__ nseg_dev, int nseg_bound,
@@ -485,7 +484,7 @@
     return hipGetLastError();
 }
 
-hipError_t launch_key_addr_flash(const KaFlashArgs& a_, int nseg_bound, bool has_set, int32_t* sched_ws, hipStream_t st) {
+hipError_t launch_key_addr_flash(const KaFlashArgs& a_, int nseg_bound, bool has_set, int32_t* sched_ws, hipStream_t st, bool slots_built) {
     KaFlashArgs a = a_;
     const KaRecLayout RL = ka_rec_layout(a.P, a.Nm, a.nR);
     if (RL.len == 0 || !sched_ws) return hipErrorInvalidValue;
@@ -497,9 +496,9 @@
     a.nslots = (int)(a.B / kFlashChunk + nseg_bound + 1);
     a.slot_seg = sched_ws;
     a.counter = sched_ws + a.nslots;
-    hipError_t e = hipMemsetAsync(sched_ws, 0xFF, ((size_t)a.nslots + 1) * sizeof(int32_t), st);
-    if (e != hipSuccess) return e;
-    {
+    if (!slots_built) {
+        hipError_t e = hipMemsetAsync(sched_ws, 0xFF, ((size_t)a.nslots + 1) * sizeof(int32_t), st);
+        if (e != hipSuccess) return e;
         const int blocks = nseg_bound < 256 * 64 ? (nseg_bound + 255) / 256 : 64;
         ka_flash_slots_kernel<<<blocks > 0 ? blocks : 1, 256, 0, st>>>(a.seg_ptr, a.nseg_dev, nseg_bound, sched_ws);
         e = hipGetLastError();
diff --git a/mvin_amd/csrc/mvin_keyaddr_static.hip b/mvin_amd/csrc/mvin_keyaddr_static.hip
--- a/mvin_amd/csrc/mvin_keyaddr_static.hip
+++ b/mvin_amd/csrc/mvin_keyaddr_static.hip
@@ -1,6 +1,7 @@
 #include <cstdlib>
 #include <utility>
 
+#include "mvin_entity_dot.h"
 #include "mvin_kernels.h"
 
 namespace mvin {
@@ -739,16 +740,7 @@
 }
 
 __global__ __launch_bounds__(256) void entity_dot_kernel(const float* __restrict__ E, const float* __restrict__ w, int n, int D, float* __restrict__ out) {
-    const int lane = threadIdx.x & 63, g = lane >> 4, c = lane & 15;
-    const int64_t row = ((int64_t)blockIdx.x * 4 + (threadIdx.x >> 6)) * 4 + g;
-    float s = 0.f;
-    if (row < n)
-        for (int d = 4 * c; d < D; d += 64) {
-            const float4 e4 = *reinterpret_cast<const float4*>(E + row * D + d), w4 = *reinterpret_cast<const float4*>(w + d);
-            s = fmaf(e4.x, w4.x, fmaf(e4.y, w4.y, fmaf(e4.z, w4.z, fmaf(e4.w, w4.w, s))));
-        }
-    s = group_sum(s, 4);
-    if (row < n && c == 0) out[row] = s;
+    entity_dot_rows<1>(E, w, n, D, out, blockIdx.x);
 }
 
 __global__ void transpose_blocks_kernel(const float* __restrict__ R, int D, float* __restrict__ RT) {
diff --git a/mvin_amd/csrc/mvin_workspaces.h b/mvin_amd/csrc/mvin_workspaces.h
--- a/mvin_amd/csrc/mvin_workspaces.h
+++ b/mvin_amd/csrc/mvin_workspaces.h
@@ -93,6 +93,9 @@
     MVIN_WS_FN size_t elems() const { return pair_index() + B; }
     MVIN_WS_FN size_t flash_sched() const { return counters(); }
     MVIN_WS_FN bool flash_sched_fits(size_t need) const { return need <= sort_elems(); }
+    MVIN_WS_FN size_t seg_user_used() const { return B < n_user ? B : n_user; }
+    MVIN_WS_FN size_t scan_sched() const { return seg_user() + seg_user_used(); }
+    MVIN_WS_FN bool scan_sched_fits(size_t need) const { return scan_sched() + need <= seg_ptr(); }
 };
 
 }
```

After: 584.6 million. No clear change (-0.1%).
